# olivesgatech/R3D

Measured on AMD Instinct MI355X. Metric: training clips/sec (RGB+Depth fusion, DARai) at 1/2/4/8 GPUs; effective-rank match, higher is better.
Workload: dtype f32 (depth products: bf16x3 split on the bf16 matrix cores, fp32 accumulate)

## Files before the change

### include/r3d_hip.h

```cpp
#ifndef R3D_HIP_H
#define R3D_HIP_H

#include <stdint.h>

#ifdef __cplusplus
extern "C" {
#endif

#define R3D_ABI_VERSION 2

#define R3D_OK 0
#define R3D_EINVAL (-1)
#define R3D_EALIGN (-2)
#define R3D_ENORCCL (-3)
#define R3D_ERCCL_BASE (-100)

int r3d_abi_version(void);
int r3d_build_info(char* buf, int cap);

int r3d_allreduce_flat(float* buf, int64_t count, void* comm, void* stream);

#define R3D_GEMM_NT 0
#define R3D_GEMM_NN 1
#define R3D_GEMM_TN 2

typedef struct r3d_gemm_desc {
    const float* A; const float* B; float* C;
    int32_t layout, M, N, K;
    int32_t lda, ldb, ldc;
    const float* a_add; int32_t a_add_mod, a_add_ld, a_row_xor;
    const float* b_add; int32_t b_add_mod, b_add_ld;
    const float* bias;
    float* pre_out; int32_t ldpre;
    int32_t act;
    const uint8_t* drop_mask; int32_t lddrop; float drop_scale;
    const float* aux; int32_t ldaux, mul;
    const float* res1; int32_t ldr1;
    const float* res2; int32_t ldr2;
    float alpha; int32_t accumulate;
    float* bias_grad;
    int32_t c_row_xor;
    int32_t splitk, k_per_split; float* partial;
    int32_t tile;
    int32_t vec;
    float* adam_m; float* adam_v; const float* adam_lr; const int64_t* adam_step;
    float adam_beta1, adam_beta2, adam_eps, adam_wd, adam_gscale;
    int32_t prec;
} r3d_gemm_desc;

int r3d_gemm_f32(const r3d_gemm_desc* d, void* stream);
int r3d_splitk_reduce(const r3d_gemm_desc* d, void* stream);
int64_t r3d_gemm_partial_floats(int32_t M, int32_t N, int32_t splitk);
int r3d_gemm_bf3_nt_pair(const r3d_gemm_desc* first, const r3d_gemm_desc* second, void* stream);
int r3d_gemm_plan(r3d_gemm_desc* d);
int r3d_gemm_grouped_prepare(r3d_gemm_desc* descs, int n, int tile, int32_t* prefix);
int r3d_gemm_grouped_launch(const r3d_gemm_desc* dev_descs, const int32_t* dev_prefix, const int32_t* host_prefix, int n,
                            int total_tiles, int layout, int tile, void* stream);

int r3d_layernorm_fwd(const float* x, int ldx, int nsplit, const float* bias, float* pre_out, const float* gamma,
                      const float* beta, float* y, int ldy, float* mean, float* rstd, float* pair_out, int rows, int H,
                      int relu, void* stream);
int64_t r3d_layernorm_bwd_ws_floats(int rows, int H);
int r3d_layernorm_bwd(const float* dy, int lddy, int pair_in, const float* dy2, int lddy2, const float* x, int ldx,
                      const float* mean,
                      const float* rstd, const float* gamma, const float* beta, int relu, const float* add1, int ldadd1,
                      const float* add2, int ldadd2, float* dx, int lddx, float* dx2, int lddx2,
                      const uint8_t* drop_mask, int lddrop, float drop_scale, float* dgamma, float* dbeta, float* ws,
                      int rows, int H, int defer_finalize, void* stream);
int r3d_layernorm_bwd_finalize(const float* ws, int rows, int H, float* dgamma, float* dbeta, void* stream);
typedef struct r3d_ln_fwd_job {
    const float* x; int32_t ldx, nsplit; const float* bias; float* pre_out;
    const float* gamma; const float* beta; float* y; int32_t ldy; float* mean; float* rstd;
    float* pair_out; int32_t rows, H, relu;
} r3d_ln_fwd_job;
typedef struct r3d_ln_bwd_job {
    const float* dy; int32_t lddy, pair_in; const float* dy2; int32_t lddy2;
    const float* x; int32_t ldx; const float* mean; const float* rstd; const float* gamma; const float* beta; int32_t relu;
    const float* add1; int32_t ldadd1; const float* add2; int32_t ldadd2;
    float* dx; int32_t lddx;
    float* dx2; int32_t lddx2; const uint8_t* drop_mask; int32_t lddrop; float drop_scale;
    float* dgamma; float* dbeta; float* ws;
    int32_t rows, H, rows_per_block, nblocks;
} r3d_ln_bwd_job;
int r3d_layernorm_fwd_multi(const r3d_ln_fwd_job* jobs, int njobs, void* stream);
int r3d_layernorm_bwd_multi(r3d_ln_bwd_job* jobs, int njobs, void* stream);
typedef struct r3d_mha_bwd_job {
    const float* q; int32_t ldq; const float* k; int32_t ldk; const float* v; int32_t ldv;
    const float* probs; const uint8_t* drop_mask; float drop_scale;
    const float* d_o; int32_t lddo; float* dq; int32_t lddq; float* dk; int32_t lddk; float* dv; int32_t lddv;
    int32_t B, heads, Lq, Lk, dh;
} r3d_mha_bwd_job;
int r3d_layernorm_bwd_multi_mha(r3d_ln_bwd_job* jobs, int njobs, const r3d_mha_bwd_job* mha, void* stream);
typedef struct r3d_ln_finalize_job { const float* ws; float* dgamma; float* dbeta; int32_t rows, H; } r3d_ln_finalize_job;
int r3d_layernorm_bwd_finalize_batched(const r3d_ln_finalize_job* dev_jobs, int njobs, int max_H, void* stream);
int64_t r3d_colsum_ws_floats(int rows, int cols);
int r3d_colsum(const float* x, int ld, int rows, int cols, float* out, float* ws, int accumulate, void* stream);
int r3d_rowmod_sum(const float* x, int ld, int rows, int cols, int mod, float* out, int ldo, int accumulate,
                   void* stream);

typedef struct r3d_rowsum_job { const float* src1; const float* src2; float* dst; int32_t ld1, ld2, ldd, rows, cols, mod; } r3d_rowsum_job;
int r3d_rowmod_sum_batched(const r3d_rowsum_job* dev_jobs, int njobs, int max_cols, int max_mod, void* stream);
int r3d_tick(int64_t* a, int64_t* b, void* stream);
int r3d_add_rowbcast(const float* x, int ldx, const float* add, int ldadd, int mod, float* out, int ldo, int rows, int cols,
                     void* stream);

typedef struct r3d_gemm_ln_job {
    const float* A; int32_t lda;
    const float* W; int32_t ldw;
    const float* bias;
    const uint8_t* drop_mask; int32_t lddrop; float drop_scale;
    const float* res1; int32_t ldr1;
    const float* res2; int32_t ldr2;
    float* pre_out; int32_t ldpre;
    const float* gamma; const float* beta;
    float* y; int32_t ldy; float* mean; float* rstd;
    float* pair_out;
    int32_t M, K;
} r3d_gemm_ln_job;
int r3d_gemm_ln_supported(int M, int K, int H);
int r3d_gemm_ln_fwd(const r3d_gemm_ln_job* jobs, int njobs, int H, void* stream);
typedef struct r3d_mha_job {
    const float* q; int32_t ldq; const float* k; int32_t ldk; const float* v; int32_t ldv;
    const uint8_t* key_padding_mask; const int64_t* key_label; int32_t pad_idx;
    float* probs; const uint8_t* drop_mask; float drop_scale; float* o; int32_t ldo;
    int32_t B, heads, Lq, Lk, dh;
} r3d_mha_job;
int r3d_gemm_ln_mha_supported(int heads, int Lq, int Lk, int dh);
int r3d_gemm_ln_mha_fwd(const r3d_gemm_ln_job* jobs, int njobs, int H, const r3d_mha_job* mha, void* stream);

typedef struct r3d_fuser_chain_fwd_args {
    const float* x0; const float* h1;
    const float* wv; const float* wproj; const float* bproj; const float* g2; const float* be2;
    const float* w1; const float* b1; const float* w2; const float* b2; const float* gf; const float* bef;
    const float* pos; const float* wkv; const float* bkv; const float* wseg; const float* bseg;
    float* vsw; float* x1; float* h2; float* m2; float* r2; float* u; float* f1; float* x3; float* y; float* mf; float* rf;
    float* fused; float* seg; float* cakv;
    const float* qpos; const float* w_in; const float* b_in; const float* w_out; const float* b_out; const float* g1;
    const float* be1; const float* wq; const float* bq;
    const uint8_t* drop_sa; const uint8_t* drop_d1; float drop_scale;
    float* sa_qkv; float* p_sa; float* sa_o; float* t1_pre; float* t1; float* m1; float* r1; float* caq;
    int32_t N, S, K, H, add_xres, B, Q, heads;
    uint64_t* timeline;
    const uint16_t* pl_wv; const uint16_t* pl_wproj; const uint16_t* pl_w1; const uint16_t* pl_w2; const uint16_t* pl_wkv;
    const uint16_t* pl_wseg;
} r3d_fuser_chain_fwd_args;
typedef struct r3d_plane_job {
    const float* src; uint16_t* dst; int32_t ld, N, K, transposed, first_block, pad_;
} r3d_plane_job;
int64_t r3d_weight_plane_elems(int N, int K);
int r3d_weight_planes(const r3d_plane_job* jobs_device, int njobs, int total_blocks, void* stream);
int r3d_fuser_chain_supported(int N, int H, int K, int B, int Q, int heads);
int r3d_fuser_chain_fwd(const r3d_fuser_chain_fwd_args* a, void* stream);
typedef struct r3d_fuser_chain_bwd_args {
    const float* d_cakv; const float* d_seg; const float* d_extra; const float* wkv; const float* wseg;
    const float* x3; const float* mf; const float* rf; const float* gf;
    const float* w2; const float* u; const float* w1; const float* x1; const float* m2; const float* r2; const float* g2;
    const float* wproj; const float* wv; const float* x0; const float* m1; const float* r1; const float* g1n;
    const uint8_t* drop_x0; const float* m_rgb; const float* m_dep; const float* rgb; const float* dep_pre;
    const float* mean_d; const float* rstd_d; const float* lnd_g; const float* lnd_b;
    float* d_fused; float* d_x3; float* d_u; float* d_h2; float* d_x1; float* d_v; float* d_h1; float* d_rgb_pre;
    float* d_dep_pre; float* part_nf; float* part_n2; float* part_n1; float* part_dep;
    const float* d_caq; const float* d_t1_res; const float* wq; const float* t1_pre; const float* m1d; const float* r1d;
    const float* g1d; const uint8_t* drop_d1; const float* w_out; const float* sa_qkv; const float* p_sa;
    const uint8_t* drop_sa; const float* w_in;
    float* caqin; float* t1pre_out; float* sap; float* sao; float* saqkv; float* sain; float* part_d1;
    float drop_scale;
    int32_t N, S, K, H, add_xres, B, Q, heads;
    uint64_t* timeline;
    const uint16_t* pl_wkv_t; const uint16_t* pl_wseg_t; const uint16_t* pl_w2_t; const uint16_t* pl_w1_t;
    const uint16_t* pl_wproj_t; const uint16_t* pl_wv_t;
} r3d_fuser_chain_bwd_args;
int r3d_fuser_chain_bwd(const r3d_fuser_chain_bwd_args* a, void* stream);

int r3d_token_exchange3_fwd(const float* xa, const float* xb, const float* xc, const float* mask, const uint8_t* drop_mask,
                            float drop_scale, float* x0, int N, int C, void* stream);
int r3d_token_exchange3_bwd(const float* dx0, const float* mask, const uint8_t* drop_mask, float drop_scale, float* da, float* db,
                            float* dc, int N, int C, void* stream);
int r3d_attn3_fwd(const float* qkv, float* probs, float* out, int N, int C, int heads, void* stream);
int r3d_attn3_bwd(const float* qkv, const float* d_out, float* d_qkv, int N, int C, int heads, void* stream);
int r3d_triple_mean_fwd(const float* y, float* out, int N, int C, void* stream);
int r3d_triple_mean_bwd(const float* d_out, float* dy, int N, int C, void* stream);

int r3d_colabssum(const float* x, int ld, int rows, int cols, double* out, void* stream);
int r3d_token_select(const float* score_f, const double* score_sum, double count, int nvec, int C, int k,
                     int64_t* idx_out, float* mask_out, int* used_serial, void* stream);
int r3d_token_exchange_fwd(const float* rgb, const float* dep, const float* mask_rgb, const float* mask_dep, float* x0,
                           const uint8_t* drop_mask, float drop_scale, int N, int H, void* stream);
int r3d_token_exchange_bwd(const float* dx0, const float* rgb, const float* mask_rgb, const float* mask_dep,
                           const uint8_t* drop_mask, float drop_scale, float* d_rgb_pre, float* d_dep, int N, int H,
                           void* stream);

int r3d_mha_core_fwd(const float* q, int ldq, const float* k, int ldk, const float* v, int ldv,
                     const uint8_t* key_padding_mask, const int64_t* key_label, int pad_idx, float* probs,
                     const uint8_t* drop_mask, float drop_scale, float* o, int ldo, int B, int heads, int Lq, int Lk,
                     int dh, void* stream);
int r3d_mha_core_bwd(const float* q, int ldq, const float* k, int ldk, const float* v, int ldv, const float* probs,
                     const uint8_t* drop_mask, float drop_scale, const float* d_o, int lddo, float* dq, int lddq, float* dk,
                     int lddk, float* dv, int lddv, int B, int heads, int Lq, int Lk, int dh, void* stream);

#define R3D_DEC_FWD_NPTRS 57
int r3d_decoder_fused_supported(int S, int Q, int H, int heads);
int r3d_decoder_layer_fwd(const void* const* ptrs, int nptrs, int B, int S, int Q, int H, int heads, int pad_idx,
                          float drop_scale, int n_head_out, void* stream);

int r3d_embed_fuse_fwd(const float* rgb_src, int ns_r, const float* bias_r, const float* dep_src, int ns_d,
                       const float* bias_d, const float* lnd_gamma, const float* lnd_beta, const float* mask_rgb,
                       const float* mask_dep, const uint8_t* drop_mask, float drop_scale, const float* ln1_gamma,
                       const float* ln1_beta, float* rgb_out, float* dep_pre_out, float* mean_d, float* rstd_d,
                       float* dep_out, float* x0, float* h1, float* m1, float* r1, int N, int H, void* stream);
int r3d_embed_fuse_fwd_planes(const float* rgb_src, int ns_r, const float* bias_r, const float* dep_src, int ns_d,
                              const float* bias_d, const float* lnd_gamma, const float* lnd_beta, const float* mask_rgb,
                              const float* mask_dep, const uint8_t* drop_mask, float drop_scale, const float* ln1_gamma,
                              const float* ln1_beta, float* rgb_out, float* dep_pre_out, float* mean_d, float* rstd_d,
                              float* dep_out, float* x0, float* h1, float* m1, float* r1, int N, int H,
                              const r3d_plane_job* jobs_device, int njobs, int total_blocks, void* stream);
int r3d_embed_fuse_bwd(const float* d_h1, const float* x0, const float* m1, const float* r1, const float* ln1_gamma,
                       const float* add1, const float* add2, const uint8_t* drop_mask, float drop_scale,
                       const float* mask_rgb, const float* mask_dep, const float* rgb, const float* dep_pre,
                       const float* mean_d, const float* rstd_d, const float* lnd_gamma, const float* lnd_beta,
                       float* d_rgb_pre, float* d_dep_pre, float* ws_n1, float* ws_dep, int N, int H, void* stream);

int r3d_bn_stats(const float* x_rgb, const float* x_dep, float* run_mean_rgb, float* run_var_rgb, int64_t* nbt_rgb,
                 float* run_mean_dep, float* run_var_dep, int64_t* nbt_dep, const float* gamma_rgb, const float* gamma_dep,
                 float* mean, float* rstd, float* absgamma, int N, int C, int training, float momentum, void* stream);
int r3d_bn_blend_fwd(const float* rgb, const float* dep, const float* mean, const float* rstd, const float* gamma_rgb,
                     const float* beta_rgb, const float* gamma_dep, const float* beta_dep, const float* alpha,
                     const float* mask_rgb, const float* mask_dep, const uint8_t* drop_mask, float drop_scale,
                     const float* ln1_gamma, const float* ln1_beta, float* x0, float* h1, float* m1, float* r1, int N, int C,
                     void* stream);
int r3d_bn_blend_bwd(const float* d_h1, const float* x0, const float* m1, const float* r1, const float* ln1_gamma,
                     const float* add1, const uint8_t* drop_mask, float drop_scale, const float* rgb, const float* dep,
                     const float* mean, const float* rstd, const float* gamma_rgb, const float* beta_rgb,
                     const float* gamma_dep, const float* beta_dep, const float* alpha, const float* mask_rgb,
                     const float* mask_dep, float* t_drb, float* t_drbx, float* t_ddb, float* t_ddbx, float* t_dal,
                     float* ws_n1, int N, int C, void* stream);
int r3d_bn_bwd_apply(const float* rgb, const float* dep, const float* mean, const float* rstd, const float* gamma_rgb,
                     const float* gamma_dep, const float* t_drb, const float* t_ddb, const float* dgamma_rgb,
                     const float* dbeta_rgb, const float* dgamma_dep, const float* dbeta_dep, float* d_rgb_pre, float* d_dep,
                     int N, int C, int training, void* stream);
int r3d_bn_sync_pack(const float* mean, const float* rstd, int N, int C, float* out, void* stream);
int r3d_bn_sync_finalize(const float* all, int world, int n_local, int C, float* mean, float* rstd, float* run_mean_rgb,
                         float* run_var_rgb, int64_t* nbt_rgb, float* run_mean_dep, float* run_var_dep, int64_t* nbt_dep,
                         float* nfrac, float momentum, void* stream);

int r3d_decoder_tail_fwd(const float* x, const float* g3, const float* b3, const float* gF, const float* bF,
                         const float* w_head, const float* b_head, int n_head, float* t3, float* m3, float* r3, float* tgtF,
                         float* mF, float* rF, float* out, int ld_out, int rows, int H, void* stream);
int r3d_decoder_tail_bwd(const float* d_out, int ld_dout, const float* w_head, int n_head, const float* t3, const float* mF,
                         const float* rF, const float* gF, const float* x, const float* m3, const float* r3, const float* g3,
                         const uint8_t* drop_mask, float drop_scale, float* dx, float* dx2, float* dgF, float* dbF,
                         float* dg3, float* db3, float* wsF, float* ws3, int rows, int H, void* stream);

int r3d_losses_fwd_bwd(const float* seg_logits, int ld_seg, const float* act_logits, int ld_act, const float* dur,
                       int ld_dur, const int64_t* past_label, const int64_t* target, const float* target_dur, int B, int S,
                       int Q, int K, int pad_idx, int exclude_idx, int val_mode, const float* dur_den, float grad_scale,
                       float* d_seg, int ld_dseg, float* d_act, int ld_dact, float* d_dur, int ld_ddur, float* loss_out,
                       int64_t* counts, float* ws, int64_t* tick_a, int64_t* tick_b, void* stream);
int64_t r3d_losses_ws_floats(int B, int S, int Q);

typedef struct r3d_tail_losses_args {
    const float* x; const float* g3; const float* b3; const float* gF; const float* bF;
    const float* w_head; const float* b_head; int n_head;
    float* t3; float* m3; float* r3; float* tgtF; float* mF; float* rF; float* out; int ld_out; int H;
    const float* seg; int ld_seg; const int64_t* past_label; const int64_t* target; const float* target_dur;
    int B, S, Q, K, pad_idx, exclude_idx; const float* dur_den; float grad_scale;
    float* d_seg; int ld_dseg; float* d_out; int ld_dout; float* loss_out; int64_t* counts; int64_t* tick_a; int64_t* tick_b;
    const uint8_t* drop; float drop_scale; float* dx; float* dx2; float* wsF; float* ws3;
    int defer_finalize;
} r3d_tail_losses_args;
int r3d_decoder_tail_losses_supported(int H, int n_head, int Q, int rows);
int r3d_decoder_tail_losses(const r3d_tail_losses_args* a, float* ws, void* stream);

typedef struct r3d_decoder_chain_args {
    const float* caq; const float* cakv; const int64_t* key_label; float* p_ca; const uint8_t* drop_ca; float* ca_o;
    const float* wo; const float* bo; const uint8_t* drop_d2; const float* t1; float* t2_pre; const float* g2; const float* be2;
    float* t2; float* m2; float* r2; const float* w1; const float* b1; const uint8_t* drop_ff; float* ff1;
    const float* w2; const float* b2; const uint8_t* drop_d3; float* t3_pre;
    const float* d_t3pre; const float* d_ff2; float* d_ff1; float* d_t2pre; float* d_cap; float* d_cao; float* d_caq;
    float* d_cakv; float* part_d2;
    float drop_scale;
    int32_t pad_idx, B, S, H, Q, heads, phases;
    uint64_t* timeline;
    const uint16_t* pl_wo; const uint16_t* pl_w1; const uint16_t* pl_w2; const uint16_t* pl_w2_t; const uint16_t* pl_w1_t;
    const uint16_t* pl_wo_t;
} r3d_decoder_chain_args;
int r3d_decoder_chain_supported(int H, int Q, int heads, int S);
int r3d_decoder_chain(const r3d_decoder_chain_args* d, const r3d_tail_losses_args* tail, float* ws, void* stream);

int r3d_adamw_flat(float* p, const float* g, float* m, float* v, int64_t n, const float* lr, const int64_t* step,
                   float beta1, float beta2, float eps, float weight_decay, float grad_scale, void* stream);
int r3d_adamw_flat_dropout(float* p, const float* g, float* m, float* v, int64_t n, const float* lr, const int64_t* step,
                           float beta1, float beta2, float eps, float weight_decay, float grad_scale, uint8_t* mask,
                           int64_t n_mask, float p_drop, uint64_t seed, const int64_t* offset, void* stream);
typedef struct r3d_loss_finalize_job {
    const float* part; int32_t B, S, Q, has_seg;
    const float* dur_den;
    float* loss_out; int64_t* counts;
    double* acc_loss; int64_t* acc_counts;
} r3d_loss_finalize_job;
int r3d_losses_finalize(const r3d_loss_finalize_job* job, void* stream);
int r3d_adamw_flat_fin(float* p, const float* g, float* m, float* v, int64_t n, const float* lr, const int64_t* step,
                       float beta1, float beta2, float eps, float weight_decay, float grad_scale,
                       const r3d_loss_finalize_job* fin, void* stream);
int r3d_adamw_flat_dropout_fin(float* p, const float* g, float* m, float* v, int64_t n, const float* lr, const int64_t* step,
                               float beta1, float beta2, float eps, float weight_decay, float grad_scale, uint8_t* mask,
                               int64_t n_mask, float p_drop, uint64_t seed, const int64_t* offset,
                               const r3d_loss_finalize_job* fin, void* stream);
int r3d_adamw_2d(float* p, const float* g, float* m, float* v, int rows, int cols, int ld, const float* lr,
                 const int64_t* step, float beta1, float beta2, float eps, float weight_decay, float grad_scale, void* stream);
int r3d_dropout_mask(uint8_t* mask, int64_t n, float p, uint64_t seed, const int64_t* offset, void* stream);

int64_t r3d_erank_lds_bytes(int R, int C);
int r3d_erank_jacobi(const float* x, int ld, int64_t batch_stride, int batch, int R, int C, int gram, float* sigma,
                     float* af_t, float* stats, int max_sweeps, void* stream);
int r3d_erank_blocked_sizes(int R, int C, int max_sweeps, int64_t* out);
int r3d_erank_blocked(const float* x, int ld, int R, int C, float* sigma, float* af_t, int* ctrl, float* stats,
                      int max_sweeps, void* stream);
int r3d_erank_blocked_t(const float* x, int ld, int x_transposed, int R, int C, float* sigma, float* af_t, int* ctrl,
                        float* stats, int max_sweeps, void* stream);
int r3d_erank_bwd_coef(const float* sigma, const float* stats, const float* gout, float* coef, int C, int max_rank,
                       void* stream);
int r3d_scale_rows(float* x, int ld, int rows, int cols, const float* coef, void* stream);
int r3d_erank_bwd_coef2(const float* sigma, const float* stats, const float* gout, float* cg, float* inv, int C, int max_rank,
                        void* stream);
int r3d_erank_bwd_fix(float* w, const float* p, const float* cg, int rows, int cols, void* stream);
int64_t r3d_erank_lds_bytes_v(int R, int C);
int r3d_erank_jacobi_warm(const float* x, int ld, int64_t batch_stride, int batch, int R, int C, int gram, float* sigma,
                          float* af_t, float* stats, int max_sweeps, const float* vt_in, float* vt_out, void* stream);
int r3d_erank_vt_polish(const float* vt_raw, const float* gv, float* vt, int64_t n, void* stream);

int r3d_posenc_fwd(const float* x, int ldx, const float* table, int ldt, int S, const uint8_t* drop, float drop_scale,
                   float* y, int ldy, int rows, int H, void* stream);
int r3d_posenc_bwd(const float* dy, int lddy, const uint8_t* drop, float drop_scale, const float* gate, int ldg, float* dx,
                   int lddx, int rows, int H, void* stream);
int r3d_avgpool_rows_fwd(const float* x, int ldx, float* y, int ldy, int B, int S, int Q, int H, void* stream);
int r3d_avgpool_rows_bwd(const float* dy, int lddy, float* dx, int lddx, int B, int S, int Q, int H, void* stream);
int r3d_embed_gather_fwd(const float* weight, int n_embed, const int64_t* idx, const float* table, int ldt, int S, float* out,
                         int ldo, int rows, int H, void* stream);
int r3d_embed_gather_bwd(const float* d_out, int ldd, const int64_t* idx, float* d_weight, int n_embed, int rows, int H,
                         void* stream);

typedef struct r3d_clip_collate_job {
    const float* rgb_pool; int64_t F_rgb, D;
    const float* depth_pool; int64_t F_dep, P;
    int64_t n_items;
    const int64_t* off_f; const int64_t* ids_f;
    const int64_t* off_d; const int64_t* ids_d;
    const int64_t* off_l; const int64_t* lab;
    const int64_t* off_q; const float* q_dur; const int64_t* q_tgt;
    const int64_t* items; int64_t B;
    int64_t S_f, S_d, S_l, S_q, pad_idx;
    float* features; float* depth; int64_t* past_label; float* trans_future_dur; int64_t* trans_future_target;
} r3d_clip_collate_job;
int r3d_clip_collate(const r3d_clip_collate_job* job, void* stream);

#ifdef __cplusplus
}
#endif
#endif
```

### r3d_amd/_lib.py

```python
import ctypes as C
import os

HERE = os.path.dirname(os.path.abspath(__file__))
LIB_PATH = os.path.join(HERE, "_build", "libr3d_hip.so")
ABI_VERSION = 2

c_float_p = C.c_void_p


class GemmDesc(C.Structure):
    _fields_ = [
        ("A", C.c_void_p), ("B", C.c_void_p), ("C", C.c_void_p),
        ("layout", C.c_int32), ("M", C.c_int32), ("N", C.c_int32), ("K", C.c_int32),
        ("lda", C.c_int32), ("ldb", C.c_int32), ("ldc", C.c_int32),
        ("a_add", C.c_void_p), ("a_add_mod", C.c_int32), ("a_add_ld", C.c_int32), ("a_row_xor", C.c_int32),
        ("b_add", C.c_void_p), ("b_add_mod", C.c_int32), ("b_add_ld", C.c_int32),
        ("bias", C.c_void_p),
        ("pre_out", C.c_void_p), ("ldpre", C.c_int32),
        ("act", C.c_int32),
        ("drop_mask", C.c_void_p), ("lddrop", C.c_int32), ("drop_scale", C.c_float),
        ("aux", C.c_void_p), ("ldaux", C.c_int32), ("mul", C.c_int32),
        ("res1", C.c_void_p), ("ldr1", C.c_int32),
        ("res2", C.c_void_p), ("ldr2", C.c_int32),
        ("alpha", C.c_float), ("accumulate", C.c_int32),
        ("bias_grad", C.c_void_p),
        ("c_row_xor", C.c_int32),
        ("splitk", C.c_int32), ("k_per_split", C.c_int32), ("partial", C.c_void_p),
        ("tile", C.c_int32),
        ("vec", C.c_int32),
        ("adam_m", C.c_void_p), ("adam_v", C.c_void_p), ("adam_lr", C.c_void_p), ("adam_step", C.c_void_p),
        ("adam_beta1", C.c_float), ("adam_beta2", C.c_float), ("adam_eps", C.c_float), ("adam_wd", C.c_float),
        ("adam_gscale", C.c_float),
        ("prec", C.c_int32),
    ]


class LnFwdJob(C.Structure):
    _fields_ = [("x", C.c_void_p), ("ldx", C.c_int32), ("nsplit", C.c_int32), ("bias", C.c_void_p), ("pre_out", C.c_void_p),
                ("gamma", C.c_void_p), ("beta", C.c_void_p), ("y", C.c_void_p), ("ldy", C.c_int32), ("mean", C.c_void_p),
                ("rstd", C.c_void_p), ("pair_out", C.c_void_p), ("rows", C.c_int32), ("H", C.c_int32), ("relu", C.c_int32)]


class LnBwdJob(C.Structure):
    _fields_ = [("dy", C.c_void_p), ("lddy", C.c_int32), ("pair_in", C.c_int32), ("dy2", C.c_void_p), ("lddy2", C.c_int32),
                ("x", C.c_void_p), ("ldx", C.c_int32), ("mean", C.c_void_p), ("rstd", C.c_void_p), ("gamma", C.c_void_p),
                ("beta", C.c_void_p), ("relu", C.c_int32), ("add1", C.c_void_p), ("ldadd1", C.c_int32), ("add2", C.c_void_p),
                ("ldadd2", C.c_int32), ("dx", C.c_void_p), ("lddx", C.c_int32), ("dx2", C.c_void_p), ("lddx2", C.c_int32),
                ("drop_mask", C.c_void_p), ("lddrop", C.c_int32), ("drop_scale", C.c_float), ("dgamma", C.c_void_p),
                ("dbeta", C.c_void_p), ("ws", C.c_void_p), ("rows", C.c_int32), ("H", C.c_int32),
                ("rows_per_block", C.c_int32), ("nblocks", C.c_int32)]


class GemmLnJob(C.Structure):
    _fields_ = [("A", C.c_void_p), ("lda", C.c_int32), ("W", C.c_void_p), ("ldw", C.c_int32), ("bias", C.c_void_p),
                ("drop_mask", C.c_void_p), ("lddrop", C.c_int32), ("drop_scale", C.c_float),
                ("res1", C.c_void_p), ("ldr1", C.c_int32), ("res2", C.c_void_p), ("ldr2", C.c_int32),
                ("pre_out", C.c_void_p), ("ldpre", C.c_int32), ("gamma", C.c_void_p), ("beta", C.c_void_p),
                ("y", C.c_void_p), ("ldy", C.c_int32), ("mean", C.c_void_p), ("rstd", C.c_void_p),
                ("pair_out", C.c_void_p), ("M", C.c_int32), ("K", C.c_int32)]


class FuserChainFwdArgs(C.Structure):
    _PTRS = ("x0 h1 wv wproj bproj g2 be2 w1 b1 w2 b2 gf bef pos wkv bkv wseg bseg vsw x1 h2 m2 r2 u f1 x3 y mf rf fused seg "
             "cakv qpos w_in b_in w_out b_out g1 be1 wq bq drop_sa drop_d1").split()
    _PTRS2 = "sa_qkv p_sa sa_o t1_pre t1 m1 r1 caq".split()
    _PLANES = "pl_wv pl_wproj pl_w1 pl_w2 pl_wkv pl_wseg".split()
    _fields_ = ([(n, C.c_void_p) for n in _PTRS] + [("drop_scale", C.c_float)] + [(n, C.c_void_p) for n in _PTRS2] +
                [(n, C.c_int32) for n in "N S K H add_xres B Q heads".split()] + [("timeline", C.c_void_p)] +
                [(n, C.c_void_p) for n in _PLANES])


class PlaneJob(C.Structure):
    _fields_ = [("src", C.c_void_p), ("dst", C.c_void_p), ("ld", C.c_int32), ("N", C.c_int32), ("K", C.c_int32),
                ("transposed", C.c_int32), ("first_block", C.c_int32), ("pad_", C.c_int32)]


class FuserChainBwdArgs(C.Structure):
    _PTRS = ("d_cakv d_seg d_extra wkv wseg x3 mf rf gf w2 u w1 x1 m2 r2 g2 wproj wv x0 m1 r1 g1n drop_x0 m_rgb m_dep rgb "
             "dep_pre mean_d rstd_d lnd_g lnd_b d_fused d_x3 d_u d_h2 d_x1 d_v d_h1 d_rgb_pre d_dep_pre part_nf part_n2 "
             "part_n1 part_dep d_caq d_t1_res wq t1_pre m1d r1d g1d drop_d1 w_out sa_qkv p_sa drop_sa w_in caqin t1pre_out "
             "sap sao saqkv sain part_d1").split()
    _PLANES = "pl_wkv_t pl_wseg_t pl_w2_t pl_w1_t pl_wproj_t pl_wv_t".split()
    _fields_ = ([(n, C.c_void_p) for n in _PTRS] + [("drop_scale", C.c_float)] +
                [(n, C.c_int32) for n in "N S K H add_xres B Q heads".split()] + [("timeline", C.c_void_p)] +
                [(n, C.c_void_p) for n in _PLANES])


class DecoderChainArgs(C.Structure):
    _PTRS = ("caq cakv key_label p_ca drop_ca ca_o wo bo drop_d2 t1 t2_pre g2 be2 t2 m2 r2 w1 b1 drop_ff ff1 w2 b2 drop_d3 "
             "t3_pre d_t3pre d_ff2 d_ff1 d_t2pre d_cap d_cao d_caq d_cakv part_d2").split()
    _fields_ = ([(n, C.c_void_p) for n in _PTRS] + [("drop_scale", C.c_float)] +
                [(n, C.c_int32) for n in "pad_idx B S H Q heads phases".split()] + [("timeline", C.c_void_p)] +
                [(n, C.c_void_p) for n in "pl_wo pl_w1 pl_w2 pl_w2_t pl_w1_t pl_wo_t".split()])


class MhaJob(C.Structure):
    _fields_ = [("q", C.c_void_p), ("ldq", C.c_int32), ("k", C.c_void_p), ("ldk", C.c_int32), ("v", C.c_void_p),
                ("ldv", C.c_int32), ("key_padding_mask", C.c_void_p), ("key_label", C.c_void_p), ("pad_idx", C.c_int32),
                ("probs", C.c_void_p), ("drop_mask", C.c_void_p), ("drop_scale", C.c_float), ("o", C.c_void_p),
                ("ldo", C.c_int32), ("B", C.c_int32), ("heads", C.c_int32), ("Lq", C.c_int32), ("Lk", C.c_int32),
                ("dh", C.c_int32)]


class MhaBwdJob(C.Structure):
    _fields_ = [("q", C.c_void_p), ("ldq", C.c_int32), ("k", C.c_void_p), ("ldk", C.c_int32), ("v", C.c_void_p),
                ("ldv", C.c_int32), ("probs", C.c_void_p), ("drop_mask", C.c_void_p), ("drop_scale", C.c_float),
                ("d_o", C.c_void_p), ("lddo", C.c_int32), ("dq", C.c_void_p), ("lddq", C.c_int32), ("dk", C.c_void_p),
                ("lddk", C.c_int32), ("dv", C.c_void_p), ("lddv", C.c_int32), ("B", C.c_int32), ("heads", C.c_int32),
                ("Lq", C.c_int32), ("Lk", C.c_int32), ("dh", C.c_int32)]


class RowsumJob(C.Structure):
    _fields_ = [("src1", C.c_void_p), ("src2", C.c_void_p), ("dst", C.c_void_p), ("ld1", C.c_int32), ("ld2", C.c_int32),
                ("ldd", C.c_int32), ("rows", C.c_int32), ("cols", C.c_int32), ("mod", C.c_int32)]


class TailLossesArgs(C.Structure):
    _fields_ = ([(n, C.c_void_p) for n in ("x", "g3", "b3", "gF", "bF", "w_head", "b_head")] + [("n_head", C.c_int32)] +
                [(n, C.c_void_p) for n in ("t3", "m3", "r3", "tgtF", "mF", "rF", "out")] +
                [("ld_out", C.c_int32), ("H", C.c_int32), ("seg", C.c_void_p), ("ld_seg", C.c_int32),
                 ("past_label", C.c_void_p), ("target", C.c_void_p), ("target_dur", C.c_void_p)] +
                [(n, C.c_int32) for n in ("B", "S", "Q", "K", "pad_idx", "exclude_idx")] +
                [("dur_den", C.c_void_p), ("grad_scale", C.c_float), ("d_seg", C.c_void_p), ("ld_dseg", C.c_int32),
                 ("d_out", C.c_void_p), ("ld_dout", C.c_int32), ("loss_out", C.c_void_p), ("counts", C.c_void_p),
                 ("tick_a", C.c_void_p), ("tick_b", C.c_void_p), ("drop", C.c_void_p), ("drop_scale", C.c_float)] +
                [(n, C.c_void_p) for n in ("dx", "dx2", "wsF", "ws3")] + [("defer_finalize", C.c_int32)])


class LossFinalizeJob(C.Structure):
    _fields_ = [("part", C.c_void_p), ("B", C.c_int32), ("S", C.c_int32), ("Q", C.c_int32), ("has_seg", C.c_int32),
                ("dur_den", C.c_void_p), ("loss_out", C.c_void_p), ("counts", C.c_void_p), ("acc_loss", C.c_void_p),
                ("acc_counts", C.c_void_p)]


class LnFinalizeJob(C.Structure):
    _fields_ = [("ws", C.c_void_p), ("dgamma", C.c_void_p), ("dbeta", C.c_void_p), ("rows", C.c_int32), ("H", C.c_int32)]


class ClipCollateJob(C.Structure):
    _fields_ = ([("rgb_pool", C.c_void_p), ("F_rgb", C.c_int64), ("D", C.c_int64),
                 ("depth_pool", C.c_void_p), ("F_dep", C.c_int64), ("P", C.c_int64), ("n_items", C.c_int64)] +
                [(n, C.c_void_p) for n in "off_f ids_f off_d ids_d off_l lab off_q q_dur q_tgt items".split()] +
                [(n, C.c_int64) for n in "B S_f S_d S_l S_q pad_idx".split()] +
                [(n, C.c_void_p) for n in "features depth past_label trans_future_dur trans_future_target".split()])


GEMM_NT, GEMM_NN, GEMM_TN = 0, 1, 2

_I, _L, _F, _P, _D = C.c_int, C.c_int64, C.c_float, C.c_void_p, C.c_double

_SIGNATURES = {
    "r3d_abi_version": ([], C.c_int),
    "r3d_build_info": ([C.c_char_p, _I], C.c_int),
    "r3d_allreduce_flat": ([_P, _L, _P, _P], C.c_int),
    "r3d_gemm_f32": ([C.POINTER(GemmDesc), _P], C.c_int),
    "r3d_splitk_reduce": ([C.POINTER(GemmDesc), _P], C.c_int),
    "r3d_gemm_partial_floats": ([C.c_int32, C.c_int32, C.c_int32], C.c_int64),
    "r3d_gemm_plan": ([C.POINTER(GemmDesc)], C.c_int),
    "r3d_gemm_grouped_prepare": ([C.POINTER(GemmDesc), _I, _I, C.POINTER(C.c_int32)], C.c_int),
    "r3d_gemm_grouped_launch": ([_P, _P, C.POINTER(C.c_int32), _I, _I, _I, _I, _P], C.c_int),
    "r3d_gemm_ln_supported": ([_I, _I, _I], C.c_int),
    "r3d_gemm_ln_fwd": ([_P, _I, _I, _P], C.c_int),
    "r3d_fuser_chain_supported": ([_I, _I, _I, _I, _I, _I], C.c_int),
    "r3d_fuser_chain_fwd": ([_P, _P], C.c_int),
    "r3d_fuser_chain_bwd": ([_P, _P], C.c_int),
    "r3d_weight_plane_elems": ([_I, _I], C.c_int64),
    "r3d_weight_planes": ([_P, _I, _I, _P], C.c_int),
    "r3d_token_exchange3_fwd": ([_P, _P, _P, _P, _P, _F, _P, _I, _I, _P], C.c_int),
    "r3d_token_exchange3_bwd": ([_P, _P, _P, _F, _P, _P, _P, _I, _I, _P], C.c_int),
    "r3d_attn3_fwd": ([_P, _P, _P, _I, _I, _I, _P], C.c_int),
    "r3d_attn3_bwd": ([_P, _P, _P, _I, _I, _I, _P], C.c_int),
    "r3d_triple_mean_fwd": ([_P, _P, _I, _I, _P], C.c_int),
    "r3d_triple_mean_bwd": ([_P, _P, _I, _I, _P], C.c_int),
    "r3d_decoder_chain_supported": ([_I, _I, _I, _I], C.c_int),
    "r3d_decoder_chain": ([_P, _P, _P, _P], C.c_int),
    "r3d_gemm_ln_mha_supported": ([_I, _I, _I, _I], C.c_int),
    "r3d_gemm_ln_mha_fwd": ([_P, _I, _I, _P, _P], C.c_int),
    "r3d_layernorm_fwd_multi": ([_P, _I, _P], C.c_int),
    "r3d_layernorm_bwd_multi": ([_P, _I, _P], C.c_int),
    "r3d_layernorm_bwd_multi_mha": ([_P, _I, _P, _P], C.c_int),
    "r3d_layernorm_bwd_finalize_batched": ([_P, _I, _I, _P], C.c_int),
    "r3d_layernorm_fwd": ([_P, _I, _I, _P, _P, _P, _P, _P, _I, _P, _P, _P, _I, _I, _I, _P], C.c_int),
    "r3d_layernorm_bwd_ws_floats": ([_I, _I], C.c_int64),
    "r3d_add_rowbcast": ([_P, _I, _P, _I, _I, _P, _I, _I, _I, _P], C.c_int),
    "r3d_layernorm_bwd": ([_P, _I, _I, _P, _I, _P, _I, _P, _P, _P, _P, _I, _P, _I, _P, _I, _P, _I, _P, _I, _P, _I, _F,
                           _P, _P, _P, _I, _I, _I, _P], C.c_int),
    "r3d_layernorm_bwd_finalize": ([_P, _I, _I, _P, _P, _P], C.c_int),
    "r3d_colsum_ws_floats": ([_I, _I], C.c_int64),
    "r3d_colsum": ([_P, _I, _I, _I, _P, _P, _I, _P], C.c_int),
    "r3d_rowmod_sum": ([_P, _I, _I, _I, _I, _P, _I, _I, _P], C.c_int),
    "r3d_rowmod_sum_batched": ([_P, _I, _I, _I, _P], C.c_int),
    "r3d_tick": ([_P, _P, _P], C.c_int),
    "r3d_colabssum": ([_P, _I, _I, _I, _P, _P], C.c_int),
    "r3d_token_select": ([_P, _P, _D, _I, _I, _I, _P, _P, _P, _P], C.c_int),
    "r3d_token_exchange_fwd": ([_P, _P, _P, _P, _P, _P, _F, _I, _I, _P], C.c_int),
    "r3d_token_exchange_bwd": ([_P, _P, _P, _P, _P, _F, _P, _P, _I, _I, _P], C.c_int),
    "r3d_mha_core_fwd": ([_P, _I, _P, _I, _P, _I, _P, _P, _I, _P, _P, _F, _P, _I, _I, _I, _I, _I, _I, _P], C.c_int),
    "r3d_mha_core_bwd": ([_P, _I, _P, _I, _P, _I, _P, _P, _F, _P, _I, _P, _I, _P, _I, _P, _I, _I, _I, _I, _I, _I, _P],
                         C.c_int),
    "r3d_decoder_fused_supported": ([_I, _I, _I, _I], C.c_int),
    "r3d_decoder_layer_fwd": ([_P, _I, _I, _I, _I, _I, _I, _I, _F, _I, _P], C.c_int),
    "r3d_embed_fuse_fwd": ([_P, _I, _P, _P, _I, _P, _P, _P, _P, _P, _P, _F, _P, _P, _P, _P, _P, _P, _P, _P, _P, _P, _P, _I, _I,
                            _P], C.c_int),
    "r3d_gemm_bf3_nt_pair": ([_P, _P, _P], C.c_int),
    "r3d_embed_fuse_fwd_planes": ([_P, _I, _P, _P, _I, _P, _P, _P, _P, _P, _P, _F, _P, _P, _P, _P, _P, _P, _P, _P, _P, _P, _P, _I,
                                   _I, _P, _I, _I, _P], C.c_int),
    "r3d_embed_fuse_bwd": ([_P, _P, _P, _P, _P, _P, _P, _P, _F, _P, _P, _P, _P, _P, _P, _P, _P, _P, _P, _P, _P, _I, _I, _P],
                           C.c_int),
    "r3d_bn_stats": ([_P] * 13 + [_I, _I, _I, _F, _P], C.c_int),
    "r3d_bn_blend_fwd": ([_P] * 12 + [_F] + [_P] * 6 + [_I, _I, _P], C.c_int),
    "r3d_bn_blend_bwd": ([_P] * 7 + [_F] + [_P] * 17 + [_I, _I, _P], C.c_int),
    "r3d_bn_bwd_apply": ([_P] * 14 + [_I, _I, _I, _P], C.c_int),
    "r3d_bn_sync_pack": ([_P, _P, _I, _I, _P, _P], C.c_int),
    "r3d_bn_sync_finalize": ([_P, _I, _I, _I] + [_P] * 9 + [_F, _P], C.c_int),
    "r3d_decoder_tail_fwd": ([_P, _P, _P, _P, _P, _P, _P, _I, _P, _P, _P, _P, _P, _P, _P, _I, _I, _I, _P], C.c_int),
    "r3d_decoder_tail_bwd": ([_P, _I, _P, _I, _P, _P, _P, _P, _P, _P, _P, _P, _P, _F, _P, _P, _P, _P, _P, _P, _P, _P, _I, _I,
                              _P], C.c_int),
    "r3d_decoder_tail_losses_supported": ([_I, _I, _I, _I], C.c_int),
    "r3d_decoder_tail_losses": ([_P, _P, _P], C.c_int),
    "r3d_losses_fwd_bwd": ([_P, _I, _P, _I, _P, _I, _P, _P, _P, _I, _I, _I, _I, _I, _I, _I, _P, _F, _P, _I, _P, _I,
                            _P, _I, _P, _P, _P, _P, _P, _P], C.c_int),
    "r3d_losses_ws_floats": ([_I, _I, _I], C.c_int64),
    "r3d_adamw_flat": ([_P, _P, _P, _P, _L, _P, _P, _F, _F, _F, _F, _F, _P], C.c_int),
    "r3d_adamw_flat_dropout": ([_P, _P, _P, _P, _L, _P, _P, _F, _F, _F, _F, _F, _P, _L, _F, C.c_uint64, _P, _P], C.c_int),
    "r3d_losses_finalize": ([_P, _P], C.c_int),
    "r3d_adamw_flat_fin": ([_P, _P, _P, _P, _L, _P, _P, _F, _F, _F, _F, _F, _P, _P], C.c_int),
    "r3d_adamw_flat_dropout_fin": ([_P, _P, _P, _P, _L, _P, _P, _F, _F, _F, _F, _F, _P, _L, _F, C.c_uint64, _P, _P, _P], C.c_int),
    "r3d_adamw_2d": ([_P, _P, _P, _P, _I, _I, _I, _P, _P, _F, _F, _F, _F, _F, _P], C.c_int),
    "r3d_dropout_mask": ([_P, _L, _F, C.c_uint64, _P, _P], C.c_int),
    "r3d_erank_lds_bytes": ([_I, _I], C.c_int64),
    "r3d_erank_jacobi": ([_P, _I, _L, _I, _I, _I, _I, _P, _P, _P, _I, _P], C.c_int),
    "r3d_erank_blocked_sizes": ([_I, _I, _I, _P], C.c_int),
    "r3d_erank_blocked": ([_P, _I, _I, _I, _P, _P, _P, _P, _I, _P], C.c_int),
    "r3d_erank_blocked_t": ([_P, _I, _I, _I, _I, _P, _P, _P, _P, _I, _P], C.c_int),
    "r3d_erank_bwd_coef": ([_P, _P, _P, _P, _I, _I, _P], C.c_int),
    "r3d_erank_bwd_coef2": ([_P, _P, _P, _P, _P, _I, _I, _P], C.c_int),
    "r3d_erank_bwd_fix": ([_P, _P, _P, _I, _I, _P], C.c_int),
    "r3d_scale_rows": ([_P, _I, _I, _I, _P, _P], C.c_int),
    "r3d_posenc_fwd": ([_P, _I, _P, _I, _I, _P, _F, _P, _I, _I, _I, _P], C.c_int),
    "r3d_posenc_bwd": ([_P, _I, _P, _F, _P, _I, _P, _I, _I, _I, _P], C.c_int),
    "r3d_avgpool_rows_fwd": ([_P, _I, _P, _I, _I, _I, _I, _I, _P], C.c_int),
    "r3d_avgpool_rows_bwd": ([_P, _I, _P, _I, _I, _I, _I, _I, _P], C.c_int),
    "r3d_embed_gather_fwd": ([_P, _I, _P, _P, _I, _I, _P, _I, _I, _I, _P], C.c_int),
    "r3d_embed_gather_bwd": ([_P, _I, _P, _P, _I, _I, _I, _P], C.c_int),
    "r3d_erank_lds_bytes_v": ([_I, _I], C.c_int64),
    "r3d_erank_jacobi_warm": ([_P, _I, _L, _I, _I, _I, _I, _P, _P, _P, _I, _P, _P, _P], C.c_int),
    "r3d_erank_vt_polish": ([_P, _P, _P, _L, _P], C.c_int),
    "r3d_clip_collate": ([C.POINTER(ClipCollateJob), _P], C.c_int),
}

EXPORTS = tuple(_SIGNATURES)

_lib = None


class R3DHipError(RuntimeError):
    pass


def load():
    global _lib
    if _lib is not None:
        return _lib
    if not os.path.exists(LIB_PATH):
        raise R3DHipError(
            f"{LIB_PATH} is missing: the HIP kernels are the only compute path of r3d_amd (no CPU/PyTorch fallback). "
            f"Build it with `python -m r3d_amd.build` (needs hipcc; cross-compiles for gfx950 without a GPU).")
    lib = C.CDLL(LIB_PATH)
    for name, (argt, rest) in _SIGNATURES.items():
        try:
            fn = getattr(lib, name)
        except AttributeError as e:
            raise R3DHipError(f"{LIB_PATH} does not export {name}: stale build, run `python -m r3d_amd.build --force`") from e
        fn.argtypes = argt
        fn.restype = rest
    v = lib.r3d_abi_version()
    if v != ABI_VERSION:
        raise R3DHipError(f"libr3d_hip.so ABI {v} != expected {ABI_VERSION}: rebuild with `python -m r3d_amd.build --force`")
    _lib = lib
    return lib


_ERR = {-1: "R3D_EINVAL (rejected argument)", -2: "R3D_EALIGN (misaligned pointer / leading dimension)",
        -3: "R3D_ENORCCL (no RCCL mapped into the process)"}


def check(rc, what):
    if rc <= -100:
        raise R3DHipError(f"{what} failed: ncclResult_t {-100 - rc} from RCCL")
    if rc != 0:
        raise R3DHipError(f"{what} failed: {_ERR.get(rc, f'hipError_t {rc}' if rc > 0 else rc)}")


def build_info():
    buf = C.create_string_buffer(128)
    check(load().r3d_build_info(buf, 128), "r3d_build_info")
    return buf.value.decode()
```

### r3d_amd/csrc/decoder_chain.hip

```cpp
#include "chain_bf3.h"
#include "mha_small.h"
#include "losses_dev.h"

namespace r3d {

constexpr int kDcBufA = 0;
constexpr int kDcBufB = kDcBufA + kFcRows * kFcP1;
constexpr int kDcBufF = kDcBufB + kFcRows * kFcP1;
constexpr int kDcWl = kDcBufF + kFcRows * kFcP4;
constexpr int kDcWlWave = 128 * kFbWP;
constexpr int kDcRed = kDcWl + 8 * kDcWlWave;
constexpr int kDcLdsFloats = kDcRed + 2 * 2 * 8 * kFcRows;
constexpr int kDcLdsBytes = kDcLdsFloats * 4;
static_assert(16 * kFcWP <= kDcWlWave && mha_small_lds_floats(16, 8) <= kDcWlWave && mha_small_bwd_lds_floats(16, 8) <= kDcWlWave,
              "wave region");
static_assert(kDcLdsBytes + (2 * 8 * (kTLHeads + 8) + 8 * 4 * 128 + 64) * 4 <= 160 * 1024, "LDS (dynamic + the tail's static arrays)");

typedef r3d_decoder_chain_args DcArgs;

__device__ __forceinline__ void dc_stage_rows(float* buf, const float* src, int row0, int tid) {
    const int r = tid >> 5, c4 = tid & 31;
    const f32x4 z = {0.f, 0.f, 0.f, 0.f};
    const f32x4 v = *reinterpret_cast<const f32x4*>(src + (size_t)(row0 + (r & 7)) * kFcH + 4 * c4);
    *reinterpret_cast<f32x4*>(buf + r * kFcP1 + 4 * c4) = r < 8 ? v : z;
// ... 123 lines not shown
    }
}

__device__ __forceinline__ void dc_bwd(const DcArgs& D, const int b, float* lds) {
    const int tid = threadIdx.x, lane = tid & 63, wave = tid >> 6;
    const int li = lane & 15, q = lane >> 4;
    float* bufA = lds + kDcBufA;
    float* bufF = lds + kDcBufF;
    float* wl = lds + kDcWl + wave * kDcWlWave;
    float* redA = lds + kDcRed;
    constexpr int H = kFcH;
    const int row0 = b * 8;
    const int c = wave * 16 + li, n0 = wave * 16;
    const bool live = q < 2;
    const f32x4 zero = {0.f, 0.f, 0.f, 0.f};
    R3D_CHAIN_MARK(D.timeline, b == 0, 10);
    FcW s0, s1;
    fb_wload(s0, D.w2 + (4 * wave + 0) * 16, 4 * H, 128, lane);
    fb_wload(s1, D.w2 + (4 * wave + 1) * 16, 4 * H, 128, lane);
    dc_stage_rows(bufA, D.d_ff2, row0, tid);
    const FcMaskSrc md2(D.drop_d2, D.g2, H), mff(D.drop_ff, D.g2, 4 * H);
    float ffv[4][4], res[4], t2pv[4], m2v[4], r2v[4];
    uint8_t kb2[4], kbf[4][4];
#pragma unroll
    for (int i = 0; i < 4; ++i) {
        const size_t r = (size_t)(row0 + ((4 * q + i) & 7));
#pragma unroll
        for (int t = 0; t < 4; ++t) {
            ffv[t][i] = D.ff1[r * (4 * H) + (4 * wave + t) * 16 + li];
            kbf[t][i] = mff.raw(r, (4 * wave + t) * 16 + li);
        }
        res[i] = D.d_t3pre[r * H + c];
        t2pv[i] = D.t2_pre[r * H + c];
        m2v[i] = D.m2[r]; r2v[i] = D.r2[r];
        kb2[i] = md2.raw(r, c);
    }
    const float g2 = D.g2[c];
    __builtin_amdgcn_sched_barrier(0);
    fb_wstore(s0, wl, lane);
    fb_wload(s0, D.w2 + (4 * wave + 2) * 16, 4 * H, 128, lane);
    __syncthreads();
    FcOp a;
    f32x4 acc0, acc1;
    R3D_CHAIN_MARK(D.timeline, b == 0, 11);
    fc_opload(a, bufA + li * kFcP1 + 4 * q);
#pragma unroll
    for (int t = 0; t < 4; ++t) {
        acc0 = zero; acc1 = zero;
        fb_chunk(a, wl, li, q, acc0, acc1);
        __builtin_amdgcn_sched_barrier(0);
        if (t == 0) { fb_wstore(s1, wl, lane); fb_wload(s1, D.w2 + (4 * wave + 3) * 16, 4 * H, 128, lane); }
        if (t == 1) { fb_wstore(s0, wl, lane); fb_wload(s0, D.w1 + n0, H, 128, lane); }
        if (t == 2) { fb_wstore(s1, wl, lane); fb_wload(s1, D.w1 + (size_t)128 * H + n0, H, 128, lane); }
        if (t == 3) { fb_wstore(s0, wl, lane); fb_wload(s0, D.w1 + (size_t)256 * H + n0, H, 128, lane); }
        __builtin_amdgcn_sched_barrier(0);
        const int cu = (4 * wave + t) * 16 + li;
#pragma unroll
        for (int i = 0; i < 4; ++i) {
            const float gv = ffv[t][i] > 0.f ? (acc0[i] + acc1[i]) * mff.keep(kbf[t][i], D.drop_scale) : 0.f;
            if (live) D.d_ff1[(size_t)(row0 + 4 * q + i) * (4 * H) + cu] = gv;
            bufF[(4 * q + i) * kFcP4 + cu] = live ? gv : 0.f;
        }
    }
    __syncthreads();
    R3D_CHAIN_MARK(D.timeline, b == 0, 12);
    acc0 = zero; acc1 = zero;
    const float* ar = bufF + li * kFcP4 + 4 * q;
    fc_opload(a, ar);
    fb_chunk(a, wl, li, q, acc0, acc1);
    __builtin_amdgcn_sched_barrier(0);
    fb_wstore(s1, wl, lane);
    fb_wload(s1, D.w1 + (size_t)384 * H + n0, H, 128, lane);
    __builtin_amdgcn_sched_barrier(0);
    fc_opload(a, ar + 128);
    fb_chunk(a, wl, li, q, acc0, acc1);
    __builtin_amdgcn_sched_barrier(0);
    fb_wstore(s0, wl, lane);
    fb_wload(s0, D.wo + n0, H, 128, lane);
    __builtin_amdgcn_sched_barrier(0);
    fc_opload(a, ar + 256);
    fb_chunk(a, wl, li, q, acc0, acc1);
    __builtin_amdgcn_sched_barrier(0);
    fb_wstore(s1, wl, lane);
    __builtin_amdgcn_sched_barrier(0);
    fc_opload(a, ar + 384);
    fb_chunk(a, wl, li, q, acc0, acc1);
    __builtin_amdgcn_sched_barrier(0);
    fb_wstore(s0, wl, lane);
    __builtin_amdgcn_sched_barrier(0);
    {
        float d[4], xh[4], g[4], gx[4], s1v[4], s2v[4];
#pragma unroll
        for (int i = 0; i < 4; ++i) {
            d[i] = live ? (acc0[i] + acc1[i]) + res[i] : 0.f;
            xh[i] = (t2pv[i] - m2v[i]) * r2v[i];
            g[i] = d[i] * g2;
            gx[i] = g[i] * xh[i];
        }
        if (live) {
            float* pp = D.part_d2 + (size_t)(2 * b + q) * (2 * H);
            pp[c] = (d[0] * xh[0] + d[1] * xh[1]) + (d[2] * xh[2] + d[3] * xh[3]);
            pp[H + c] = (d[0] + d[1]) + (d[2] + d[3]);
        }
        fb_rowsum2<4>(g, gx, redA, wave, li, q, s1v, s2v);
#pragma unroll
        for (int i = 0; i < 4; ++i) {
            const float o = r2v[i] * (g[i] - s1v[i] - xh[i] * s2v[i]);
            const size_t e = (size_t)(row0 + 4 * q + i) * H + c;
            const float ok = o * md2.keep(kb2[i], D.drop_scale);
            if (live) { D.d_t2pre[e] = o; D.d_cap[e] = ok; }
            bufA[(4 * q + i) * kFcP1 + c] = live ? ok : 0.f;
        }
    }
    __syncthreads();
    R3D_CHAIN_MARK(D.timeline, b == 0, 13);
    fc_opload(a, bufA + li * kFcP1 + 4 * q);
    acc0 = zero; acc1 = zero;
    fb_chunk(a, wl, li, q, acc0, acc1);
    if (live) {
#pragma unroll
        for (int i = 0; i < 4; ++i) D.d_cao[(size_t)(row0 + 4 * q + i) * H + c] = acc0[i] + acc1[i];
    }
    R3D_CHAIN_MARK(D.timeline, b == 0, 14);
    __syncthreads();
    {
        MhaArgs m{};
        m.q = D.caq; m.ldq = H; m.k = D.cakv; m.ldk = 2 * H; m.v = D.cakv + H; m.ldv = 2 * H;
        m.probs = D.p_ca; m.drop = D.drop_ca; m.drop_scale = D.drop_scale; m.d_o = D.d_cao; m.lddo = H;
        m.dq = D.d_caq; m.lddq = H; m.dk = D.d_cakv; m.lddk = 2 * H; m.dv = D.d_cakv + H; m.lddv = 2 * H;
        m.B = D.B; m.heads = 8; m.Lq = 8; m.Lk = D.S; m.dh = 16; m.scale = 0.25f;
        mha_bwd_small_unit<16, 8, false>(m, b * 8 + wave, wl);
    }
    R3D_CHAIN_MARK(D.timeline, b == 0, 15);
}

constexpr int kD3P1 = kFcH + 8, kD3P4 = 4 * kFcH + 8;
constexpr int kD3ImgA = 0;
constexpr int kD3ImgB = kD3ImgA + 3 * 16 * kD3P1;
constexpr int kD3ImgF = kD3ImgB + 3 * 16 * kD3P1;
constexpr int kD3ScrBytes = (kD3ImgF + 3 * 16 * kD3P4) * 2;
constexpr int kD3ScrWave = 1856;
constexpr int kD3RedBytes = kD3ScrBytes + 8 * kD3ScrWave * 4;
constexpr int kD3LdsBytes = kD3RedBytes + 2 * 2 * 8 * kFcRows * 4;
static_assert(mha_small_lds_floats(16, 8) <= kD3ScrWave && mha_small_bwd_lds_floats(16, 8) <= kD3ScrWave, "attention scratch");
static_assert(kD3LdsBytes + (2 * 8 * (kTLHeads + 8) + 8 * 4 * 128 + 64) * 4 <= 160 * 1024, "LDS (dynamic + the tail's static arrays)");

__device__ __forceinline__ void dc3_stage_rows(unsigned short* img, const float* src, int row0, int tid) {
    const int r = tid >> 5, c4 = tid & 31;
    const f32x4 z = {0.f, 0.f, 0.f, 0.f};
    const f32x4 v = *reinterpret_cast<const f32x4*>(src + (size_t)(row0 + (r & 7)) * kFcH + 4 * c4);
    bf3_store4(img, kD3P1, r, 4 * c4, r < 8 ? v : z);
}

__device__ __forceinline__ void dc3_fwd(const DcArgs& D, const int b, float* lds) {
    const int tid = threadIdx.x, lane = tid & 63, wave = tid >> 6;
    const int li = lane & 15, q = lane >> 4;
    unsigned short* img = reinterpret_cast<unsigned short*>(lds);
    unsigned short* imgA = img + kD3ImgA;
    unsigned short* imgB = img + kD3ImgB;
    unsigned short* imgF = img + kD3ImgF;
    float* scr = reinterpret_cast<float*>(reinterpret_cast<unsigned char*>(lds) + kD3ScrBytes) + wave * kD3ScrWave;
    float (*red)[8][kFcRows] = reinterpret_cast<float (*)[8][kFcRows]>(reinterpret_cast<unsigned char*>(lds) + kD3RedBytes);
    constexpr int H = kFcH;
    const int row0 = b * 8;
    const int c = wave * 16 + li;
    const bool live = q < 2;
    const f32x4 zero = {0.f, 0.f, 0.f, 0.f};
    R3D_CHAIN_MARK(D.timeline, b == 0, 0);
    Bf3B b0, b1, b2;
    bf3_bload<4>(b0, D.pl_wo, 4, wave, 0, lane);
    bf3_bload<4>(b1, D.pl_w1, 4, 4 * wave + 0, 0, lane);
    bf3_bload<4>(b2, D.pl_w1, 4, 4 * wave + 1, 0, lane);
    const FcMaskSrc md2(D.drop_d2, D.g2, H), md3(D.drop_d3, D.g2, H), mff(D.drop_ff, D.g2, 4 * H);
    float t1v[4];
    uint8_t kb2[4], kb3[4], kbf[4][4];
#pragma unroll
    for (int i = 0; i < 4; ++i) {
        const size_t r = (size_t)(row0 + ((4 * q + i) & 7));
        t1v[i] = D.t1[r * H + c];
        kb2[i] = md2.raw(r, c);
        kb3[i] = md3.raw(r, c);
#pragma unroll
        for (int t = 0; t < 4; ++t) kbf[t][i] = mff.raw(r, (4 * wave + t) * 16 + li);
    }
    const float b_o = D.bo[c], g2 = D.g2[c], be2 = D.be2[c], b_2 = D.b2[c];
    float b_1[4];
#pragma unroll
    for (int t = 0; t < 4; ++t) b_1[t] = D.b1[(4 * wave + t) * 16 + li];
    R3D_CHAIN_MARK(D.timeline, b == 0, 1);
    {
        MhaArgs m{};
        m.q = D.caq; m.ldq = H; m.k = D.cakv; m.ldk = 2 * H; m.v = D.cakv + H; m.ldv = 2 * H;
        m.key_label = D.key_label; m.pad_idx = D.pad_idx; m.probs = D.p_ca; m.drop = D.drop_ca; m.drop_scale = D.drop_scale;
        m.o = D.ca_o; m.ldo = H; m.B = D.B; m.heads = 8; m.Lq = 8; m.Lk = D.S; m.dh = 16; m.scale = 0.25f;
        mha_fwd_small_unit<16, 8, false>(m, b * 8 + wave, scr);
    }
    R3D_CHAIN_MARK(D.timeline, b == 0, 2);
    __syncthreads();
    dc3_stage_rows(imgA, D.ca_o, row0, tid);
    __syncthreads();
    R3D_CHAIN_MARK(D.timeline, b == 0, 3);
    f32x4 acc0 = zero, acc1 = zero;
    bf3_chunk<4>(imgA, kD3P1, li, q, 0, b0, acc0, acc1);
    __builtin_amdgcn_sched_barrier(0);
    bf3_bload<4>(b0, D.pl_w1, 4, 4 * wave + 2, 0, lane);
    __builtin_amdgcn_sched_barrier(0);
    float t2p[4], mean[4], rstd[4], t2v[4];
#pragma unroll
    for (int i = 0; i < 4; ++i) {
        t2p[i] = ((acc0[i] + acc1[i]) + b_o) * md2.keep(kb2[i], D.drop_scale) + t1v[i];
        if (live) D.t2_pre[(size_t)(row0 + 4 * q + i) * H + c] = t2p[i];
    }
    fc_layernorm(t2p, red, wave, li, q, mean, rstd);
#pragma unroll
    for (int i = 0; i < 4; ++i) {
        t2v[i] = (t2p[i] - mean[i]) * rstd[i] * g2 + be2;
        const int r = 4 * q + i;
        if (live) {
            D.t2[(size_t)(row0 + r) * H + c] = t2v[i];
            if (wave == 0 && li == 0) { D.m2[row0 + r] = mean[i]; D.r2[row0 + r] = rstd[i]; }
        }
        bf3_store1(imgB, kD3P1, r, c, live ? t2v[i] : 0.f);
    }
    __syncthreads();
    R3D_CHAIN_MARK(D.timeline, b == 0, 4);
#pragma unroll
    for (int t = 0; t < 4; ++t) {
        acc0 = zero; acc1 = zero;
        if (t == 0) bf3_chunk<4>(imgB, kD3P1, li, q, 0, b1, acc0, acc1);
        if (t == 1) bf3_chunk<4>(imgB, kD3P1, li, q, 0, b2, acc0, acc1);
        if (t == 2) bf3_chunk<4>(imgB, kD3P1, li, q, 0, b0, acc0, acc1);
        if (t == 3) bf3_chunk<4>(imgB, kD3P1, li, q, 0, b1, acc0, acc1);
        __builtin_amdgcn_sched_barrier(0);
        if (t == 0) bf3_bload<4>(b1, D.pl_w1, 4, 4 * wave + 3, 0, lane);
        if (t == 1) bf3_bload<4>(b2, D.pl_w2, 16, wave, 0, lane);
        if (t == 2) bf3_bload<4>(b0, D.pl_w2, 16, wave, 4, lane);
        if (t == 3) bf3_bload<4>(b1, D.pl_w2, 16, wave, 8, lane);
        __builtin_amdgcn_sched_barrier(0);
        const int cu = (4 * wave + t) * 16 + li;
#pragma unroll
        for (int i = 0; i < 4; ++i) {
            const float f = fmaxf((acc0[i] + acc1[i]) + b_1[t], 0.f) * mff.keep(kbf[t][i], D.drop_scale);
            if (live) D.ff1[(size_t)(row0 + 4 * q + i) * (4 * H) + cu] = f;
            bf3_store1(imgF, kD3P4, 4 * q + i, cu, live ? f : 0.f);
        }
    }
    __syncthreads();
    R3D_CHAIN_MARK(D.timeline, b == 0, 5);
    acc0 = zero; acc1 = zero;
    bf3_chunk<4>(imgF, kD3P4, li, q, 0, b2, acc0, acc1);
    __builtin_amdgcn_sched_barrier(0);
    bf3_bload<4>(b2, D.pl_w2, 16, wave, 12, lane);
    __builtin_amdgcn_sched_barrier(0);
    bf3_chunk<4>(imgF, kD3P4, li, q, 4, b0, acc0, acc1);
    bf3_chunk<4>(imgF, kD3P4, li, q, 8, b1, acc0, acc1);
    bf3_chunk<4>(imgF, kD3P4, li, q, 12, b2, acc0, acc1);
    if (live) {
#pragma unroll
        for (int i = 0; i < 4; ++i)
            D.t3_pre[(size_t)(row0 + 4 * q + i) * H + c] =
                ((acc0[i] + acc1[i]) + b_2) * md3.keep(kb3[i], D.drop_scale) + t2v[i];
    }
}

__device__ __forceinline__ void dc3_bwd(const DcArgs& D, const int b, float* lds) {
    const int tid = threadIdx.x, lane = tid & 63, wave = tid >> 6;
    const int li = lane & 15, q = lane >> 4;
    unsigned short* img = reinterpret_cast<unsigned short*>(lds);
    unsigned short* imgA = img + kD3ImgA;
    unsigned short* imgF = img + kD3ImgF;
    float* scr = reinterpret_cast<float*>(reinterpret_cast<unsigned char*>(lds) + kD3ScrBytes) + wave * kD3ScrWave;
    float* redA = reinterpret_cast<float*>(reinterpret_cast<unsigned char*>(lds) + kD3RedBytes);
    constexpr int H = kFcH;
    const int row0 = b * 8;
    const int c = wave * 16 + li;
    const bool live = q < 2;
    const f32x4 zero = {0.f, 0.f, 0.f, 0.f};
    R3D_CHAIN_MARK(D.timeline, b == 0, 10);
    Bf3B b0, b1, b2;
    bf3_bload<4>(b0, D.pl_w2_t, 4, 4 * wave + 0, 0, lane);
    bf3_bload<4>(b1, D.pl_w2_t, 4, 4 * wave + 1, 0, lane);
    bf3_bload<4>(b2, D.pl_w2_t, 4, 4 * wave + 2, 0, lane);
    dc3_stage_rows(imgA, D.d_ff2, row0, tid);
    const FcMaskSrc md2(D.drop_d2, D.g2, H), mff(D.drop_ff, D.g2, 4 * H);
    float ffv[4][4], res[4], t2pv[4], m2v[4], r2v[4];
    uint8_t kb2[4], kbf[4][4];
#pragma unroll
    for (int i = 0; i < 4; ++i) {
        const size_t r = (size_t)(row0 + ((4 * q + i) & 7));
#pragma unroll
        for (int t = 0; t < 4; ++t) {
            ffv[t][i] = D.ff1[r * (4 * H) + (4 * wave + t) * 16 + li];
            kbf[t][i] = mff.raw(r, (4 * wave + t) * 16 + li);
        }
        res[i] = D.d_t3pre[r * H + c];
        t2pv[i] = D.t2_pre[r * H + c];
        m2v[i] = D.m2[r]; r2v[i] = D.r2[r];
        kb2[i] = md2.raw(r, c);
    }
    const float g2 = D.g2[c];
    __syncthreads();
    R3D_CHAIN_MARK(D.timeline, b == 0, 11);
    f32x4 acc0, acc1;
#pragma unroll
    for (int t = 0; t < 4; ++t) {
        acc0 = zero; acc1 = zero;
        if (t == 0) bf3_chunk<4>(imgA, kD3P1, li, q, 0, b0, acc0, acc1);
        if (t == 1) bf3_chunk<4>(imgA, kD3P1, li, q, 0, b1, acc0, acc1);
        if (t == 2) bf3_chunk<4>(imgA, kD3P1, li, q, 0, b2, acc0, acc1);
        if (t == 3) bf3_chunk<4>(imgA, kD3P1, li, q, 0, b0, acc0, acc1);
        __builtin_amdgcn_sched_barrier(0);
        if (t == 0) bf3_bload<4>(b0, D.pl_w2_t, 4, 4 * wave + 3, 0, lane);
        if (t == 1) bf3_bload<4>(b1, D.pl_w1_t, 16, wave, 0, lane);
        if (t == 2) bf3_bload<4>(b2, D.pl_w1_t, 16, wave, 4, lane);
        if (t == 3) bf3_bload<4>(b0, D.pl_w1_t, 16, wave, 8, lane);
        __builtin_amdgcn_sched_barrier(0);
        const int cu = (4 * wave + t) * 16 + li;
#pragma unroll
        for (int i = 0; i < 4; ++i) {
            const float gv = ffv[t][i] > 0.f ? (acc0[i] + acc1[i]) * mff.keep(kbf[t][i], D.drop_scale) : 0.f;
            if (live) D.d_ff1[(size_t)(row0 + 4 * q + i) * (4 * H) + cu] = gv;
            bf3_store1(imgF, kD3P4, 4 * q + i, cu, live ? gv : 0.f);
        }
    }
    __syncthreads();
    R3D_CHAIN_MARK(D.timeline, b == 0, 12);
    acc0 = zero; acc1 = zero;
    bf3_chunk<4>(imgF, kD3P4, li, q, 0, b1, acc0, acc1);
    __builtin_amdgcn_sched_barrier(0);
    bf3_bload<4>(b1, D.pl_w1_t, 16, wave, 12, lane);
    __builtin_amdgcn_sched_barrier(0);
    bf3_chunk<4>(imgF, kD3P4, li, q, 4, b2, acc0, acc1);
    __builtin_amdgcn_sched_barrier(0);
    bf3_bload<4>(b2, D.pl_wo_t, 4, wave, 0, lane);
    __builtin_amdgcn_sched_barrier(0);
    bf3_chunk<4>(imgF, kD3P4, li, q, 8, b0, acc0, acc1);
    bf3_chunk<4>(imgF, kD3P4, li, q, 12, b1, acc0, acc1);
    {
        float d[4], xh[4], g[4], gx[4], s1v[4], s2v[4];
#pragma unroll
        for (int i = 0; i < 4; ++i) {
            d[i] = live ? (acc0[i] + acc1[i]) + res[i] : 0.f;
            xh[i] = (t2pv[i] - m2v[i]) * r2v[i];
            g[i] = d[i] * g2;
            gx[i] = g[i] * xh[i];
        }
        if (live) {
            float* pp = D.part_d2 + (size_t)(2 * b + q) * (2 * H);
            pp[c] = (d[0] * xh[0] + d[1] * xh[1]) + (d[2] * xh[2] + d[3] * xh[3]);
            pp[H + c] = (d[0] + d[1]) + (d[2] + d[3]);
        }
        fb_rowsum2<4>(g, gx, redA, wave, li, q, s1v, s2v);
#pragma unroll
        for (int i = 0; i < 4; ++i) {
            const float o = r2v[i] * (g[i] - s1v[i] - xh[i] * s2v[i]);
            const size_t e = (size_t)(row0 + 4 * q + i) * H + c;
            const float ok = o * md2.keep(kb2[i], D.drop_scale);
            if (live) { D.d_t2pre[e] = o; D.d_cap[e] = ok; }
            bf3_store1(imgA, kD3P1, 4 * q + i, c, live ? ok : 0.f);
        }
    }
    __syncthreads();
    R3D_CHAIN_MARK(D.timeline, b == 0, 13);
    acc0 = zero; acc1 = zero;
    bf3_chunk<4>(imgA, kD3P1, li, q, 0, b2, acc0, acc1);
    if (live) {
#pragma unroll
        for (int i = 0; i < 4; ++i) D.d_cao[(size_t)(row0 + 4 * q + i) * H + c] = acc0[i] + acc1[i];
    }
    R3D_CHAIN_MARK(D.timeline, b == 0, 14);
    __syncthreads();
    {
        MhaArgs m{};
        m.q = D.caq; m.ldq = H; m.k = D.cakv; m.ldk = 2 * H; m.v = D.cakv + H; m.ldv = 2 * H;
        m.probs = D.p_ca; m.drop = D.drop_ca; m.drop_scale = D.drop_scale; m.d_o = D.d_cao; m.lddo = H;
        m.dq = D.d_caq; m.lddq = H; m.dk = D.d_cakv; m.lddk = 2 * H; m.dv = D.d_cakv + H; m.lddv = 2 * H;
        m.B = D.B; m.heads = 8; m.Lq = 8; m.Lk = D.S; m.dh = 16; m.scale = 0.25f;
        mha_bwd_small_unit<16, 8, false>(m, b * 8 + wave, scr);
    }
    R3D_CHAIN_MARK(D.timeline, b == 0, 15);
}

__global__ __launch_bounds__(512) void decoder_chain_bf3_kernel(const DcArgs D, const r3d_tail_losses_args t, const LossArgs a,
                                                                float* part, unsigned* arrivals) {
    extern __shared__ __attribute__((aligned(16))) float lds[];
    __shared__ float lg[8][kTLHeads + 8];
    __shared__ float dl[8][kTLHeads + 8];
    __shared__ float red[8][4][128];
    __shared__ int is_last;
    if (threadIdx.x >= 256) __builtin_amdgcn_s_setprio(0); else __builtin_amdgcn_s_setprio(2);
    const int lane = threadIdx.x & 63, wave = threadIdx.x >> 6;
    if ((int)blockIdx.x < D.B) {
        const int b = (int)blockIdx.x;
        if (D.phases & 1) dc3_fwd(D, b, lds);
        R3D_CHAIN_MARK(D.timeline, b == 0, 6);
        if (D.phases & 2) {
            __syncthreads();
            tail_clip_body(t, a, part, b, lg, dl, red);
        }
        R3D_CHAIN_MARK(D.timeline, b == 0, 7);
        if (D.phases & 4) {
            __syncthreads();
            dc3_bwd(D, b, lds);
        }
    } else if (D.phases & 2) {
        const int u = ((int)blockIdx.x - D.B) * 8 + wave;
        if (u < a.B * a.S) losses_unit(a, part, u, lane);
    }
    if (D.phases & 2) tail_losses_finish(t, a, part, arrivals, &is_last);
}

__global__ __launch_bounds__(512) void decoder_chain_kernel(const DcArgs D, const r3d_tail_losses_args t, const LossArgs a,
                                                            float* part, unsigned* arrivals) {
    extern __shared__ __attribute__((aligned(16))) float lds[];
    if (threadIdx.x >= 256) __builtin_amdgcn_s_setprio(0); else __builtin_amdgcn_s_setprio(2);
    __shared__ float lg[8][kTLHeads + 8];
    __shared__ float dl[8][kTLHeads + 8];
    __shared__ float red[8][4][128];
    __shared__ int is_last;
    const int lane = threadIdx.x & 63, wave = threadIdx.x >> 6;
    if ((int)blockIdx.x < D.B) {
        const int b = (int)blockIdx.x;
        if (D.phases & 1) dc_fwd(D, b, lds);
        R3D_CHAIN_MARK(D.timeline, b == 0, 6);
        if (D.phases & 2) {
            __syncthreads();
            tail_clip_body(t, a, part, b, lg, dl, red);
        }
        R3D_CHAIN_MARK(D.timeline, b == 0, 7);
        if (D.phases & 4) {
            __syncthreads();
            dc_bwd(D, b, lds);
        }
    } else if (D.phases & 2) {
        const int u = ((int)blockIdx.x - D.B) * 8 + wave;
        if (u < a.B * a.S) losses_unit(a, part, u, lane);
    }
    if (D.phases & 2) tail_losses_finish(t, a, part, arrivals, &is_last);
}

}

using namespace r3d;

R3D_EXPORT int r3d_decoder_tail_losses_supported(int H, int n_head, int Q, int rows);

R3D_EXPORT int r3d_decoder_chain_supported(int H, int Q, int heads, int S) {
    return (H == kFcH && Q == 8 && heads == 8 && S > 0 && S <= 64) ? 1 : 0;
}

R3D_EXPORT int r3d_decoder_chain(const r3d_decoder_chain_args* d, const r3d_tail_losses_args* tail, float* ws, void* stream) {
    R3D_REQUIRE(d && (d->phases & 7) && !(d->phases & ~7));
    R3D_REQUIRE(r3d_decoder_chain_supported(d->H, d->Q, d->heads, d->S) && d->B > 0);
    R3D_REQUIRE(d->caq && d->cakv && d->p_ca && d->wo && d->w1 && d->w2 && d->t2_pre && d->m2 && d->r2 && d->g2 && d->ff1);
    if (d->phases & 1)
        R3D_REQUIRE(d->ca_o && d->bo && d->t1 && d->be2 && d->t2 && d->b1 && d->b2 && d->t3_pre);
    if (d->phases & 4)
        R3D_REQUIRE(d->d_t3pre && d->d_ff2 && d->d_ff1 && d->d_t2pre && d->d_cap && d->d_cao && d->d_caq && d->d_cakv && d->part_d2);
    const void* al[] = {d->caq, d->cakv, d->wo, d->w1, d->w2, d->ca_o, d->d_ff2, d->d_cao, d->d_cakv};
    for (const void* p : al)
        if (p && !r3d_aligned16(p)) return R3D_EALIGN;
    r3d_tail_losses_args t{};
    LossArgs a{};
    int grid = d->B;
    unsigned* arrivals = nullptr;
    if (d->phases & 2) {
        R3D_REQUIRE(tail && ws);
        t = *tail;
        R3D_REQUIRE(t.x && t.g3 && t.b3 && t.gF && t.bF && t.w_head && t.b_head && t.t3 && t.m3 && t.r3 && t.tgtF && t.mF && t.rF);
        R3D_REQUIRE(t.out && t.seg && t.past_label && t.target && t.target_dur && t.d_seg && t.d_out && t.loss_out && t.counts);
        R3D_REQUIRE(t.dx && t.dx2 && t.wsF && t.ws3);
        R3D_REQUIRE(t.B == d->B && t.S == d->S && t.Q == d->Q && t.H == d->H && t.K > 0 && t.n_head == t.K + 1);
        R3D_REQUIRE(t.ld_out >= t.n_head && t.ld_dout >= t.n_head && t.ld_seg >= t.K && t.ld_dseg >= t.K);
        if (!r3d_decoder_tail_losses_supported(t.H, t.n_head, t.Q, t.B * t.Q)) return R3D_EINVAL;
        if (!r3d_aligned16(ws)) return R3D_EALIGN;
        if (d->phases & 1) R3D_REQUIRE(t.x == d->t3_pre);
        if (d->phases & 4) R3D_REQUIRE(t.dx == d->d_t3pre && t.dx2 == d->d_ff2);
        a = LossArgs{t.seg, t.ld_seg, t.out, t.ld_out, t.out + t.K, t.ld_out, t.past_label, t.target, t.target_dur, t.B, t.S, t.Q,
                     t.K, t.pad_idx, t.exclude_idx, 0, t.dur_den, t.grad_scale, t.d_seg, t.ld_dseg, t.d_out, t.ld_dout,
                     t.d_out + t.K, t.ld_dout, t.loss_out, t.counts, t.tick_a, t.tick_b};
        const int units = t.B * t.S + t.B * t.Q + t.B;
        grid = t.B + r3d_cdiv(t.B * t.S, 8);
        arrivals = reinterpret_cast<unsigned*>(ws + 4 * (size_t)units);
    }
    if (d->pl_wo) {
        R3D_REQUIRE(d->pl_w1 && d->pl_w2 && d->pl_w2_t && d->pl_w1_t && d->pl_wo_t);
        hipError_t e3 = hipFuncSetAttribute((const void*)decoder_chain_bf3_kernel, hipFuncAttributeMaxDynamicSharedMemorySize,
                                            kD3LdsBytes);
        if (e3 != hipSuccess) return (int)e3;
        hipLaunchKernelGGL(decoder_chain_bf3_kernel, dim3(grid), dim3(512), (size_t)kD3LdsBytes, (hipStream_t)stream, *d, t, a, ws,
                           arrivals);
        R3D_LAUNCH_CHECK();
        return R3D_OK;
    }
    hipError_t e = hipFuncSetAttribute((const void*)decoder_chain_kernel, hipFuncAttributeMaxDynamicSharedMemorySize, kDcLdsBytes);
    if (e != hipSuccess) return (int)e;
    hipLaunchKernelGGL(decoder_chain_kernel, dim3(grid), dim3(512), (size_t)kDcLdsBytes, (hipStream_t)stream, *d, t, a, ws, arrivals);
    R3D_LAUNCH_CHECK();
    return R3D_OK;
}
```

### r3d_amd/engine.py

```python
import math

import torch

from . import ops
from ._lib import GEMM_NT, GEMM_NN, GEMM_TN

LIVE_PREFIXES = ("input_embed.", "depth_projection.", "depth_layernorm.", "pos_embedding", "query_embed.",
                 "fuser.blocks.", "fuser.norm.", "transformer.decoder.", "fc_seg.", "fc.", "fc_len.")
EXCLUDE_CLASS_IDX = 47
DROP_P = 0.1


BN_LIVE_PREFIXES = ("fuser.alpha", "fuser.bn_rgb.", "fuser.bn_depth.")


def is_live(name):
    return name.startswith(LIVE_PREFIXES)


BWD_BF3_MAX_K = 32


def fuser_chain_shape_ok(B, S, H, K, Q, heads, bn=False):
    return bool(not bn and H // heads == 16 and ops.fuser_chain_supported(B * S, H, K, B, Q, heads))


def decoder_chain_shape_ok(B, S, H, Q, heads, L):
    return bool(L == 1 and H // heads == 16 and B * Q <= 1024 and ops.decoder_chain_supported(H, Q, heads, S))


def bwd_chain_bf3(chain_bf3, K):
    return bool(chain_bf3 and K <= BWD_BF3_MAX_K)


def tail_in_decoder_chain(B, H, K, Q):
    return ops.tail_losses_supported(H, K + 1, Q, B * Q)


class ParamArena:

    def __init__(self, named_params, device, extra_live=()):
        named = list(named_params)
        self.is_live = lambda n: is_live(n) or (bool(extra_live) and n.startswith(tuple(extra_live)))
        live = [(n, p) for n, p in named if self.is_live(n)]
        dead = [(n, p) for n, p in named if not self.is_live(n)]

        def key(item):
            n, p = item
            if n == "depth_projection.weight":
                return (3, 0)
            if n in ("fc.weight", "fc_len.weight"):
                return (0, 0 if n == "fc.weight" else 1)
            if n in ("fc.bias", "fc_len.bias"):
                return (2, 0 if n == "fc.bias" else 1)
            if n == "pos_embedding":
                return (2, 9)
            return (1, 0) if p.numel() % 4 == 0 else (2, 2)
        order = sorted(range(len(live)), key=lambda i: (key(live[i]), i))
        live = [live[i] for i in order]
        self.offsets, off = {}, 0
        for n, p in live:
            if n in ("depth_projection.weight", "pos_embedding"):
                off = (off + 3) // 4 * 4
            self.offsets[n] = (off, p.numel(), tuple(p.shape))
            off += p.numel()
        self.n_live = (off + 3) // 4 * 4
        off = self.n_live
        for n, p in dead:
            off = (off + 3) // 4 * 4
            self.offsets[n] = (off, p.numel(), tuple(p.shape))
            off += p.numel()
        self.n_total = (off + 3) // 4 * 4
        big0 = self.offsets["depth_projection.weight"][0] if "depth_projection.weight" in self.offsets else self.n_live
        self.bucket_small = (0, big0)
        self.bucket_big = (big0, self.n_live)
        self.params = torch.zeros(self.n_total, dtype=torch.float32, device=device)
        self.grads = torch.zeros(self.n_live, dtype=torch.float32, device=device)
        self.exp_avg = torch.zeros(self.n_live, dtype=torch.float32, device=device)
        self.exp_avg_sq = torch.zeros(self.n_live, dtype=torch.float32, device=device)
        self.live_names = [n for n, _ in live]
        with torch.no_grad():
            for n, p in named:
                o, k, shp = self.offsets[n]
                self.params[o:o + k].copy_(p.detach().reshape(-1).to(device=device, dtype=torch.float32))
                p.data = self.params[o:o + k].view(shp)
                p.grad = None

    def p(self, name):
        o, k, shp = self.offsets[name]
        return self.params[o:o + k].view(shp)

    def g(self, name):
        o, k, shp = self.offsets[name]
        return self.grads[o:o + k].view(shp)

    def attach_grads(self, named_params):
        for n, p in named_params:
            p.grad = self.g(n) if self.is_live(n) else None


class _Shape:

    def __init__(self, eng, B, S, train):
        dev, H, Q, K, L, heads = eng.device, eng.H, eng.Q, eng.K, eng.L, eng.heads
        N, BQ = B * S, B * Q
        f = lambda *s: torch.empty(*s, dtype=torch.float32, device=dev)
        self.B, self.S, self.N, self.BQ = B, S, N, BQ
        self.rgb, self.dep, self.dep_pre = f(N, H), f(N, H), f(N, H)
        self.mean_d, self.rstd_d = f(N), f(N)
        if eng.bn:
            self.bn_mean, self.bn_rstd, self.bn_absg = f(2, H), f(2, H), f(2, H)
            self.bn_idx = torch.empty(2, max(1, int(H * 0.1)), dtype=torch.int64, device=dev)
        self.sums = torch.empty(2, H, dtype=torch.float64, device=dev)
        self.idx = torch.empty(2, H // 4, dtype=torch.int64, device=dev)
        self.mask = f(2, H)
        self.x0, self.h1, self.vsw, self.x1, self.h2 = f(2 * N, H), f(2 * N, H), f(2 * N, H), f(2 * N, H), f(2 * N, H)
        self.u, self.f1 = f(2 * N, 4 * H), f(2 * N, 4 * H)
        self.x3, self.y = f(2 * N, H), f(2 * N, H)
        self.m1, self.r1, self.m2, self.r2, self.mf, self.rf = f(2 * N), f(2 * N), f(2 * N), f(2 * N), f(2 * N), f(2 * N)
        self.fused = f(N, H)
        self.tgt0 = torch.zeros(BQ, H, dtype=torch.float32, device=dev)
        self.layers = []
        for _ in range(L):
            d = dict(sa_qkv=f(BQ, 3 * H), sa_o=f(BQ, H), p_sa=f(B, heads, Q, Q), t1_pre=f(BQ, H),
                     t1=f(BQ, H), m1=f(BQ), r1=f(BQ), caq=f(BQ, H), cakv=f(N, 2 * H), ca_o=f(BQ, H),
                     p_ca=f(B, heads, Q, S), t2_pre=f(BQ, H), t2=f(BQ, H), m2=f(BQ), r2=f(BQ), ff1=f(BQ, 4 * H),
                     t3_pre=f(BQ, H), t3=f(BQ, H), m3=f(BQ), r3=f(BQ))
            self.layers.append(d)
        self.tgtF, self.mF, self.rF = f(BQ, H), f(BQ), f(BQ)
        self.actdur = f(BQ, K + 1)
        self.seg = f(N, K)
        self.loss = f(4)
        self.tables = {}
        self.loss_ws = torch.zeros(ops.losses_ws_floats(B, S, eng.Q), dtype=torch.float32, device=dev)
        self.counts = torch.zeros(4, dtype=torch.int64, device=dev)
        if train:
            self.d_actdur, self.d_seg = torch.zeros(BQ, K + 1, dtype=torch.float32, device=dev), f(N, K)
            self.d_tgtF, self.d_t = f(BQ, H), f(BQ, H)
            self.glayers = [dict(t3pre=f(BQ, H), ff2=f(BQ, H), ff1=f(BQ, 4 * H), t2=f(BQ, H), t2pre=f(BQ, H), cap=f(BQ, H),
                                 cao=f(BQ, H), caq=f(BQ, H), cakv=f(N, 2 * H), caqin=f(BQ, H), t1pre=f(BQ, H), sap=f(BQ, H),
                                 sao=f(BQ, H), saqkv=f(BQ, 3 * H), sain=f(BQ, H), t2b=f(BQ, H)) for _ in range(L)]
            self.d_fused, self.d_fused2 = f(N, H), f(N, H)
            lnw = lambda rows: f(max(ops.layernorm_bwd_ws_floats(rows, H), 4))
            self.lnp = dict(final=lnw(BQ), nf=lnw(2 * N), n2=lnw(2 * N), n1=lnw(2 * N), dep=lnw(N))
            self.lnp_seam = dict(n1=f(2 * N * H), dep=f(2 * N * H))
            for l in range(L):
                self.lnp.update({f"d3_{l}": lnw(BQ), f"d2_{l}": lnw(BQ), f"d1_{l}": lnw(BQ)})
            self.d_x3, self.d_u, self.d_h1, self.d_h2, self.d_x1, self.d_v, self.d_x0 = (
                f(2 * N, H), f(2 * N, 4 * H), f(2 * N, H), f(2 * N, H), f(2 * N, H), f(2 * N, H), f(2 * N, H))
            self.d_rgb_pre, self.d_dep, self.d_dep_pre = f(N, H), f(N, H), f(N, H)
            self.d_h2b = f(2 * N, H)
            if eng.bn:
                self.bn_terms = [f(N, H) for _ in range(5)]
            sizes = dict(x0=2 * N * H)
            for l in range(L):
                sizes.update({f"sa_p{l}": B * heads * Q * Q, f"ca_p{l}": B * heads * Q * S, f"d1_{l}": BQ * H,
                              f"d2_{l}": BQ * H, f"d3_{l}": BQ * H, f"ff_{l}": BQ * 4 * H})
            tot = sum((v + 15) // 16 * 16 for v in sizes.values())
            self.drop_pool = torch.ones(tot, dtype=torch.uint8, device=dev)
            self.drop, o = {}, 0
            for k, v in sizes.items():
                self.drop[k] = self.drop_pool[o:o + v]
                o += (v + 15) // 16 * 16


class FusionEngine:
    def __init__(self, module, device):
        self.module = module
        self.device = torch.device(device)
        assert self.device.type == "cuda", "the HIP engine needs an MI355X device (there is no CPU path)"
        ops._lib.load()
        self.H, self.Q, self.K = module.hidden_dim, module.n_query, module.n_class
        self.heads, self.L = module.n_head, module.num_decoder_layers
        self.dh = self.H // self.heads
        self.pad_idx = module.src_pad_idx
        self.P, self.D = module.depth_projection.in_features, module.input_embed.in_features
        assert self.H % 8 == 0 and self.H % self.heads == 0
        self.bn = hasattr(module.fuser, "bn_rgb")
        self.arena = ParamArena(list(module.named_parameters()), self.device, BN_LIVE_PREFIXES if self.bn else ())
        self.ws = ops.GemmWorkspace(self.device)
        self._sel = {}
        self.ws_side = ops.GemmWorkspace(self.device)
        self.side = torch.cuda.Stream(self.device)
        self.side2 = torch.cuda.Stream(self.device)
        self.ws_side2 = ops.GemmWorkspace(self.device)
        self.auto_side_stream = True
        self.use_side_stream = False
        self.use_fused_decoder = False
        self.use_fused_tail = True
        self.defer_tail = False
        self.use_paired_launches = True
        self.use_gemm_ln = True
        self.use_fuser_chain = True
        self.use_decoder_chain = True
        self.chain_bf3 = True
        self._planes = None
        self.overlap_planes = False
        self.overlap_param_tail = False
        self.ride_planes = True
        self._planes_rode = False
        self.fuse_depth_adamw = True
        self.pair_embeddings = True
        self._planes_forked = False
        self._tail_pending = False
        self._overlap_tail_now = False
        self.defer_loss_reduce = False
        self.loss_acc = None
        self.fold_rowsums = True
        self.ride_attention = True
        self.ride_attention_bwd = False
        self.split_k4h = False
        self.depth_prec = 1
        self.use_fused_embed = not self.bn
        self.dropout_enabled = bool(getattr(module, "r3d_dropout_enabled", True))
        self.erank_weight = 0.0
        self.erank_warm_start = False
        self.erank_max_sweeps = 16
        self.erank_side_stream = True
        self.er_stream = torch.cuda.Stream(self.device)
        self.ws_er = ops.GemmWorkspace(self.device)
        self._er_pending = False
        self.shapes = {}
        self.train_mask = None
        self.drop_seed = 0x5EED
        self.drop_offset = torch.zeros(1, dtype=torch.int64, device=self.device)
        self.lr_t = torch.zeros(1, dtype=torch.float32, device=self.device)
        self.step_t = torch.zeros(1, dtype=torch.int64, device=self.device)
        self._lr_host = None
        self.dur_den = None
        self.score_allreduce = None
        self.bn_sync = None
        self.grad_hook = None
        self.tp = None
        self._fw = None
        self.last = None
        self._adam = None
        self._drop_ready = None
        self.pos_grad_rows = 0
        a = self.arena
        K, H = self.K, self.H
        o_w = a.offsets["fc.weight"][0]
        self.w_head = a.params[o_w:o_w + (K + 1) * H].view(K + 1, H)
        self.gw_head = a.grads[o_w:o_w + (K + 1) * H].view(K + 1, H)
        o_b = a.offsets["fc.bias"][0]
        assert a.offsets["fc_len.weight"][0] == o_w + K * H and a.offsets["fc_len.bias"][0] == o_b + K
        self.b_head = a.params[o_b:o_b + K + 1]
        self.gb_head = a.grads[o_b:o_b + K + 1]

    def _shape(self, B, S, train):
        key = (B, S, bool(train))
        if key not in self.shapes:
            self.shapes[key] = _Shape(self, B, S, train)
        return self.shapes[key]

    def _train_masks(self, B, S):
        if self.train_mask is None:
            C = self.H
            sc = torch.full((2, C), 1.0 / (B * S * C), dtype=torch.float32, device=self.device)
            idx = torch.empty(2, C // 4, dtype=torch.int64, device=self.device)
            mask = torch.empty(2, C, dtype=torch.float32, device=self.device)
            ops.token_select(C // 4, idx, mask, score_f=sc)
            self.train_mask = (idx, mask)
        return self.train_mask

    def forward(self, feats, depth, labels, mode="train", training=False, need_grad=True, bn_training=None):
        self.forward_begin(feats, depth, labels, mode, training, need_grad)
        self._fw["bn_training"] = training if bn_training is None else bn_training
        if self._fw["tp"] is not None:
            self._fw["tp"].exchange_forward(self._fw["w"])
        return self.forward_finish()

    def forward_begin(self, feats, depth, labels, mode="train", training=False, need_grad=True):
        a, H = self.arena, self.H
        B, S = feats.shape[0], feats.shape[1]
        N = B * S
        assert feats.is_cuda and depth.is_cuda and feats.dtype == torch.float32 and depth.dtype == torch.float32
        x_rgb = feats.reshape(N, -1)
        x_dep = depth.reshape(N, -1)
        assert x_rgb.shape[1] == self.D and x_dep.shape[1] == self.P, (x_rgb.shape, x_dep.shape, self.D, self.P)
        assert x_rgb.is_contiguous() and x_dep.is_contiguous()
        w = self._shape(B, S, need_grad)
        self._loss_pending = None
        self._erank_join()
        drop = training and need_grad and self.dropout_enabled
        if drop:
            if self._drop_ready is w:
                self._drop_ready = None
            else:
                ops.dropout_mask(w.drop_pool, DROP_P, self.drop_seed, self.drop_offset)
        tp = self.tp if (self.tp is not None and need_grad) else None
        seam = self.use_fused_embed and mode == "train" and H <= 1024
        self._join_tail()
        if (self.overlap_planes and self.chain_bf3 and self.L == 1 and (self.use_fuser_chain or self.use_decoder_chain) and
                self._chain_shape_ok(w)):
            self.side.wait_stream(torch.cuda.current_stream())
            with torch.cuda.stream(self.side):
                self.chain_planes().refresh()
            self._planes_forked = True
        rgb_done = None
        dr = d = None
        if seam and tp is None and self.depth_prec == 1 and self.pair_embeddings:
            pr = ops.gemm_bf3_nt_pair(x_dep, a.p("depth_projection.weight"), w.dep_pre, self.ws,
                                      x_rgb, a.p("input_embed.weight"), w.rgb, self.ws_side)
            if pr is not None:
                d, dr = pr
        if dr is None:
            dr = ops.gemm(GEMM_NT, x_rgb, a.p("input_embed.weight"), w.rgb, bias=a.p("input_embed.bias"), act=1,
                          ws=self.ws_side if seam else self.ws, defer_reduce=seam, prec=self.depth_prec)
        slabs_r = self.ws_side.buf if (seam and dr.splitk > 1) else None
        if d is not None:
            pass
        elif tp is None:
            d = ops.gemm(GEMM_NT, x_dep, a.p("depth_projection.weight"), w.dep_pre, bias=a.p("depth_projection.bias"),
                         ws=self.ws, defer_reduce=True, prec=self.depth_prec)
        else:
            tp.partial_forward(w, x_dep, self.ws)
        slabs = self.ws.buf if (d is not None and d.splitk > 1) else None
        self._fw = dict(w=w, x_rgb=x_rgb, x_dep=x_dep, labels=labels, mode=mode, drop=drop, d=d, tp=tp, B=B, S=S,
                        slabs=slabs, seam=seam, dr=dr, slabs_r=slabs_r, rgb_done=rgb_done)

    def forward_finish(self):
        fw = self._fw
        w, x_rgb, x_dep, labels, mode, drop, d, tp = (fw[k] for k in ("w", "x_rgb", "x_dep", "labels", "mode", "drop", "d",
                                                                       "tp"))
        B, S = fw["B"], fw["S"]
        a, H, Q, K, heads, dh = self.arena, self.H, self.Q, self.K, self.heads, self.dh
        N, BQ = B * S, B * Q
        dsc = 1.0 / (1.0 - DROP_P)
        dm = (lambda k: w.drop[k]) if drop else (lambda k: None)
        key_labels = None
        if mode == "train":
            assert labels.dtype == torch.int64 and labels.is_cuda and labels.is_contiguous()
            key_labels = labels
        main = torch.cuda.current_stream()
        multi = self._multi_stream()
        s2 = self.side2 if multi else main
        ws2 = self.ws_side2 if multi else self.ws
        qpos = a.p("query_embed.weight")
        pos = a.p("pos_embedding")[0, :S]

        def sa_block(l, tgt_in, wsx):
            c, pl = w.layers[l], f"transformer.decoder.layers.{l}."
            ops.gemm(GEMM_NT, tgt_in, a.p(pl + "self_attn.in_proj_weight"), c["sa_qkv"], a_add=qpos, a_add_mod=Q,
                     bias=a.p(pl + "self_attn.in_proj_bias"), ws=wsx)
            ops.mha_core_fwd(c["sa_qkv"][:, :H], c["sa_qkv"][:, H:2 * H], c["sa_qkv"][:, 2 * H:], c["p_sa"], c["sa_o"], B,
                             heads, Q, Q, dh, drop_mask=dm(f"sa_p{l}"), drop_scale=dsc)
            if self._gln(BQ, H):
# ... 108 lines not shown
        if not paired:
            self._erank_fork(w)
        if paired:
            pass
        elif not fused_dec:
            if not hasattr(w, "fwd_group"):
                wi0 = a.p("transformer.decoder.layers.0.multihead_attn.in_proj_weight")
                bi0 = a.p("transformer.decoder.layers.0.multihead_attn.in_proj_bias")
                w.fwd_group = ops.GemmGroup(GEMM_NT, [
                    dict(a=w.fused, b=a.p("fc_seg.weight"), c=w.seg, bias=a.p("fc_seg.bias")),
                    dict(a=w.fused, b=wi0[H:], c=w.layers[0]["cakv"], bias=bi0[H:], a_add=pos, a_add_mod=S)],
                    tile=1 if H < 256 else 2)
            w.fwd_group.launch()
        else:
            ops.gemm(GEMM_NT, w.fused, a.p("fc_seg.weight"), w.seg, bias=a.p("fc_seg.bias"), ws=self.ws)
        self.last_drop_flag = bool(drop)
        if fused_dec:
            self._decoder_fused(w, key_labels, drop, dsc)
        else:
            self._decoder_unfused(w, key_labels, dm, dsc, multi, main, s2, sa_block, paired)
        if self._planes_forked:
            main.wait_stream(self.side)
            self._planes_forked = False
        self._planes_rode = False
        er = self.erank_weight != 0.0 and hasattr(w, "glayers")
        if er and not w.__dict__.get("_er_forked", False):
            self._erank_forward(w)
        w._er_forked = False
        self.last = dict(w=w, x_rgb=x_rgb, x_dep=x_dep, mask=mask, idx=idx, drop=drop, mode=mode, tp=tp, seam=seam, erank=er,
                         paired=paired, bn_training=bool(fw.get("bn_training", False)))
        return dict(seg=w.seg.view(B, S, K), action=w.actdur[:, :K].view(B, Q, K), duration=w.actdur[:, K].view(B, Q))

    def _erank_fork(self, w):
        if self.erank_weight == 0.0 or not hasattr(w, "glayers") or not self.erank_side_stream:
            return
        self.er_stream.wait_stream(torch.cuda.current_stream())
        with torch.cuda.stream(self.er_stream):
            self._erank_forward(w)
        w._er_forked = True
        self._er_pending = True

    def _erank_join(self):
        if self._er_pending:
            torch.cuda.current_stream().wait_stream(self.er_stream)
            self._er_pending = False

    def _erank_forward(self, w):
        N, H = w.N, self.H
        if not hasattr(w, "er_sigma"):
            f = lambda *s: torch.empty(*s, dtype=torch.float32, device=self.device)
            w.er_gout = f(1)
            w.er_blk = None
            if ops.erank_fits(N, H):
                w.er_sigma, w.er_stats, w.er_af = f(1, H), f(1, 4), f(1, H, N)
                w.er_vt = torch.eye(H, dtype=torch.float32, device=self.device)
                w.er_vraw, w.er_vg, w.er_gv, w.er_xw = f(H, H), f(H, H), f(H, H), f(N, H)
            else:
                w.er_flip = N < H
                R, Cc = (H, N) if w.er_flip else (N, H)
                w.er_blk = ops.ErankBlockedBufs(R, Cc, self.device, max_sweeps=self.erank_max_sweeps)
                w.er_sigma, w.er_stats = w.er_blk.sigma.view(1, Cc), w.er_blk.stats.view(1, 4)
        if w.er_blk is not None:
            ops.erank_blocked_into(w.fused, w.er_blk, transposed=w.er_flip)
        elif self.erank_warm_start and ops.erank_fits_warm(N, H):
            wsx = self.ws_er
            ops.gemm(GEMM_NT, w.fused, w.er_vt, w.er_xw, ws=wsx)
            ops.erank_jacobi_warm(w.er_xw, w.er_sigma, w.er_stats, w.er_vraw, vt_in=w.er_vt, af_t=w.er_af)
            ops.gemm(GEMM_NT, w.er_vraw, w.er_vraw, w.er_vg, ws=wsx)
            ops.gemm(GEMM_NN, w.er_vg, w.er_vraw, w.er_gv, ws=wsx)
            ops.erank_vt_polish(w.er_vraw, w.er_gv, w.er_vt)
        else:
            ops.erank_jacobi(w.fused, w.er_sigma, w.er_stats, af_t=w.er_af)

    def _erank_backward(self, w, ws, dst=None):
        from .erank import ErankBackward
        if not hasattr(w, "er_bwd"):
            w.er_bwd = ErankBackward(w.N, self.H, w.er_blk is not None and w.er_flip, self.device)
        w.er_gout.fill_(-float(self.erank_weight))
        A = w.er_blk.af_t if w.er_blk is not None else w.er_af[0]
        w.er_bwd.run(w.fused, A, w.er_sigma[0], w.er_stats[0], w.er_gout, dst if dst is not None else w.d_fused2,
                     dst is None, ws)

    def erank_value(self):
        self._erank_join()
        return self.last["w"].er_stats[0, 0]

    def chain_planes(self):
        if self._planes is None:
            a, H = self.arena, self.H
            pre, pl = "fuser.blocks.0.", "transformer.decoder.layers.0."
            wi = a.p(pl + "multihead_attn.in_proj_weight")
            W = dict(wv=a.p(pre + "attn.qkv.weight")[2 * H:], wproj=a.p(pre + "attn.proj.weight"), w1=a.p(pre + "mlp.mlp.0.weight"),
                     w2=a.p(pre + "mlp.mlp.2.weight"), wkv=wi[H:], wseg=a.p("fc_seg.weight"),
                     dec_wo=a.p(pl + "multihead_attn.out_proj.weight"), dec_w1=a.p(pl + "linear1.weight"),
                     dec_w2=a.p(pl + "linear2.weight"))
            ent = {}
            for k, w_ in W.items():
                ent["pl_" + k] = (w_, False)
                ent["pl_" + k + "_t"] = (w_, True)
            self._planes = ops.WeightPlanes(ent, self.device)
        return self._planes

    def _multi_stream(self):
        return bool(self.use_side_stream or (self.auto_side_stream and self.H >= 512 and self.tp is None and
                                             self.grad_hook is None))

    def _planes_refresh(self):
        if self._planes_forked:
            torch.cuda.current_stream().wait_stream(self.side)
            self._planes_forked = False
        elif self._planes_rode:
            pass
        else:
            self.chain_planes().refresh()

    def _join_tail(self):
        if self._tail_pending:
            torch.cuda.current_stream().wait_stream(self.side)
            self._tail_pending = False

    def _chain_shape_ok(self, w):
        return fuser_chain_shape_ok(w.B, w.S, self.H, self.K, self.Q, self.heads, self.bn)

    def _chain_ok(self, w):
        return bool(self.use_fuser_chain and self._chain_shape_ok(w))

    def _dec_chain_ok(self, w):
        return bool(self.use_decoder_chain and decoder_chain_shape_ok(w.B, w.S, self.H, self.Q, self.heads, self.L))

    def _dec_chain(self, w, drop):
        bf3 = bool(self.chain_bf3)
        key = ("dec_chain", bool(drop), bf3)
        if bf3 and not (self.use_fuser_chain and self._chain_shape_ok(w)):
            self._planes_refresh()
        if key not in w.tables:
            pls = self.chain_planes() if bf3 else None
            dpl = None
            if pls is not None:
                dpl = dict(pl_wo=pls.ptr("pl_dec_wo"), pl_w1=pls.ptr("pl_dec_w1"), pl_w2=pls.ptr("pl_dec_w2"),
                           pl_w2_t=pls.ptr("pl_dec_w2_t"), pl_w1_t=pls.ptr("pl_dec_w1_t"), pl_wo_t=pls.ptr("pl_dec_wo_t"))
            a, H = self.arena, self.H
            c, pl = w.layers[0], "transformer.decoder.layers.0."
            dk = (lambda k: w.drop[k]) if drop else (lambda k: None)
            gl = w.glayers[0] if hasattr(w, "glayers") else None
            g = (lambda k: gl[k]) if gl is not None else (lambda k: None)
            w.tables[key] = ops.DecoderChain(
                caq=c["caq"], cakv=c["cakv"], p_ca=c["p_ca"], drop_ca=dk("ca_p0"), ca_o=c["ca_o"],
                wo=a.p(pl + "multihead_attn.out_proj.weight"), bo=a.p(pl + "multihead_attn.out_proj.bias"), drop_d2=dk("d2_0"),
                t1=c["t1"], t2_pre=c["t2_pre"], g2=a.p(pl + "norm2.weight"), be2=a.p(pl + "norm2.bias"), t2=c["t2"], m2=c["m2"],
                r2=c["r2"], w1=a.p(pl + "linear1.weight"), b1=a.p(pl + "linear1.bias"), drop_ff=dk("ff_0"), ff1=c["ff1"],
                w2=a.p(pl + "linear2.weight"), b2=a.p(pl + "linear2.bias"), drop_d3=dk("d3_0"), t3_pre=c["t3_pre"],
                d_t3pre=g("t3pre"), d_ff2=g("ff2"), d_ff1=g("ff1"), d_t2pre=g("t2pre"), d_cap=g("cap"), d_cao=g("cao"),
                d_caq=g("caq"), d_cakv=g("cakv"), part_d2=w.lnp["d2_0"] if gl is not None else None,
                drop_scale=1.0 / (1.0 - DROP_P), pad_idx=self.pad_idx, B=w.B, S=w.S, H=H, Q=self.Q, heads=self.heads, planes=dpl)
        return w.tables[key]

    def _gln(self, rows, K):
        return self.use_gemm_ln and ops.gemm_ln_supported(rows, K, self.H)

    def _forward_paired(self, w, fw, dm, dsc, drop, wv, pre, qpos, pos):
        a, H, Q, S, B, BQ, heads, dh = self.arena, self.H, self.Q, w.S, w.B, w.BQ, self.heads, self.dh
        c, pl = w.layers[0], "transformer.decoder.layers.0."
        if self._chain_ok(w):
            bf3 = bool(self.chain_bf3)
            key = ("fwd_chain", bool(drop), bf3)
            if bf3:
                self._planes_refresh()
            if key not in w.tables:
                pls = self.chain_planes() if bf3 else None
                wi, bi = a.p(pl + "multihead_attn.in_proj_weight"), a.p(pl + "multihead_attn.in_proj_bias")
                w.tables[key] = ops.FuserChainFwd(
                    x0=w.x0, h1=w.h1, wv=wv, wproj=a.p(pre + "attn.proj.weight"), bproj=a.p(pre + "attn.proj.bias"),
                    g2=a.p(pre + "norm2.weight"), be2=a.p(pre + "norm2.bias"), w1=a.p(pre + "mlp.mlp.0.weight"),
                    b1=a.p(pre + "mlp.mlp.0.bias"), w2=a.p(pre + "mlp.mlp.2.weight"), b2=a.p(pre + "mlp.mlp.2.bias"),
                    gf=a.p("fuser.norm.weight"), bef=a.p("fuser.norm.bias"), pos=pos.contiguous(), wkv=wi[H:], bkv=bi[H:],
                    wseg=a.p("fc_seg.weight"), bseg=a.p("fc_seg.bias"), vsw=w.vsw, x1=w.x1, h2=w.h2, m2=w.m2, r2=w.r2, u=w.u,
                    f1=w.f1, x3=w.x3, y=w.y, mf=w.mf, rf=w.rf, fused=w.fused, seg=w.seg, cakv=c["cakv"],
                    qpos=qpos, w_in=a.p(pl + "self_attn.in_proj_weight"), b_in=a.p(pl + "self_attn.in_proj_bias"),
                    w_out=a.p(pl + "self_attn.out_proj.weight"), b_out=a.p(pl + "self_attn.out_proj.bias"),
                    g1=a.p(pl + "norm1.weight"), be1=a.p(pl + "norm1.bias"), wq=wi[:H], bq=bi[:H],
                    drop_sa=dm("sa_p0"), drop_d1=dm("d1_0"), drop_scale=dsc, sa_qkv=c["sa_qkv"], p_sa=c["p_sa"],
                    sa_o=c["sa_o"], t1_pre=c["t1_pre"], t1=c["t1"], m1=c["m1"], r1=c["r1"], caq=c["caq"],
                    N=w.N, S=S, K=self.K, H=H, add_xres=0 if self.bn else 1, B=B, Q=Q, heads=heads,
                    planes={k: pls.ptr(k) for k in pls.keys if not k.endswith("_t") and "dec_" not in k} if pls is not None else None)
            w.tables[key].launch()
            self._erank_fork(w)
            return
        key = ("fwd_pairs", bool(drop))
        if key not in w.tables:
            wi, bi = a.p(pl + "multihead_attn.in_proj_weight"), a.p(pl + "multihead_attn.in_proj_bias")
            t = 1 if H < 256 else 2
            g1 = ops.GemmGroup(GEMM_NT, [
                dict(a=w.h1, b=wv, c=w.vsw, c_row_xor=1),
                dict(a=w.tgt0, b=a.p(pl + "self_attn.in_proj_weight"), c=c["sa_qkv"], a_add=qpos, a_add_mod=Q,
                     bias=a.p(pl + "self_attn.in_proj_bias"))], tile=t)
            g2 = ops.GemmGroup(GEMM_NT, [
                dict(a=w.h2, b=a.p(pre + "mlp.mlp.0.weight"), c=w.f1, bias=a.p(pre + "mlp.mlp.0.bias"), act=2, pre_out=w.u),
                dict(a=c["sa_o"], b=a.p(pl + "self_attn.out_proj.weight"), c=c["t1_pre"],
                     bias=a.p(pl + "self_attn.out_proj.bias"), drop_mask=self._dm2(dm("d1_0"), BQ, H), drop_scale=dsc)],
                tile=t)
            g3 = ops.GemmGroup(GEMM_NT, [
                dict(a=w.fused, b=a.p("fc_seg.weight"), c=w.seg, bias=a.p("fc_seg.bias")),
                dict(a=w.fused, b=wi[H:], c=c["cakv"], bias=bi[H:], a_add=pos, a_add_mod=S),
                dict(a=c["t1"], b=wi[:H], c=c["caq"], a_add=qpos, a_add_mod=Q, bias=bi[:H])], tile=t)
            w.tables[key] = (g1, g2, g3)
        g1, g2, g3 = w.tables[key]
        g1.launch()
        gln = self._gln(2 * w.N, H) and self._gln(2 * w.N, 4 * H) and self._gln(BQ, 0)
        sa = dict(q=c["sa_qkv"][:, :H], k=c["sa_qkv"][:, H:2 * H], v=c["sa_qkv"][:, 2 * H:], probs=c["p_sa"], o=c["sa_o"], B=B,
                  heads=heads, Lq=Q, Lk=Q, dh=dh, drop_mask=dm("sa_p0"), drop_scale=dsc)
        ride = gln and self.ride_attention and ops.gemm_ln_mha_supported(heads, Q, Q, dh)
        if gln:
            ops.gemm_ln_fwd([dict(a=w.vsw, w=a.p(pre + "attn.proj.weight"), bias=a.p(pre + "attn.proj.bias"), res1=w.x0,
                                  pre=w.x1, gamma=a.p(pre + "norm2.weight"), beta=a.p(pre + "norm2.bias"), y=w.h2,
                                  mean=w.m2, rstd=w.r2)], mha=sa if ride else None)
        else:
            ops.gemm(GEMM_NT, w.vsw, a.p(pre + "attn.proj.weight"), w.x1, bias=a.p(pre + "attn.proj.bias"), res1=w.x0,
                     ws=self.ws)
        if not ride:
            ops.mha_core_fwd(sa["q"], sa["k"], sa["v"], sa["probs"], sa["o"], B, heads, Q, Q, dh, drop_mask=sa["drop_mask"],
                             drop_scale=dsc)
        if not gln:
            ops.layernorm_fwd(w.x1, a.p(pre + "norm2.weight"), a.p(pre + "norm2.bias"), w.h2, w.m2, w.r2)
        g2.launch()
        if gln:
            ops.gemm_ln_fwd([
                dict(a=w.f1, w=a.p(pre + "mlp.mlp.2.weight"), bias=a.p(pre + "mlp.mlp.2.bias"), res1=w.x1,
                     res2=None if self.bn else w.x0, pre=w.x3, gamma=a.p("fuser.norm.weight"),
                     beta=a.p("fuser.norm.bias"), y=w.y, mean=w.mf, rstd=w.rf, pair_out=w.fused),
                dict(a=None, pre=c["t1_pre"], gamma=a.p(pl + "norm1.weight"), beta=a.p(pl + "norm1.bias"), y=c["t1"],
                     mean=c["m1"], rstd=c["r1"])])
        else:
            ops.gemm(GEMM_NT, w.f1, a.p(pre + "mlp.mlp.2.weight"), w.x3, bias=a.p(pre + "mlp.mlp.2.bias"), res1=w.x1,
                     res2=None if self.bn else w.x0, ws=self.ws)
            ops.layernorm_fwd_multi([
                dict(x=c["t1_pre"], gamma=a.p(pl + "norm1.weight"), beta=a.p(pl + "norm1.bias"), y=c["t1"], mean=c["m1"],
                     rstd=c["r1"]),
                dict(x=w.x3, gamma=a.p("fuser.norm.weight"), beta=a.p("fuser.norm.bias"), y=w.y, mean=w.mf, rstd=w.rf,
                     pair_out=w.fused)])
        self._erank_fork(w)
        g3.launch()

    def _decoder_unfused(self, w, key_labels, dm, dsc, multi, main, s2, sa_block, paired=False):
        a, H, Q, K, heads, dh = self.arena, self.H, self.Q, self.K, self.heads, self.dh
        B, S, N, BQ = w.B, w.S, w.N, w.BQ
        pos = a.p("pos_embedding")[0, :S]
        tgt = None
        for l in range(self.L):
            c, pl = w.layers[l], f"transformer.decoder.layers.{l}."
            wi, bi = a.p(pl + "multihead_attn.in_proj_weight"), a.p(pl + "multihead_attn.in_proj_bias")
            if l > 0:
                ops.gemm(GEMM_NT, w.fused, wi[H:], c["cakv"], a_add=pos, a_add_mod=S, bias=bi[H:], ws=self.ws)
            if l == 0:
                if multi:
                    main.wait_stream(s2)
            else:
                sa_block(l, tgt, self.ws)
            w._dec_deferred = False
            if paired and self._dec_chain_ok(w):
                drop_now = self.last_drop_flag
                w._tail_done = False
                w._tail_deferred = bool(self.use_fused_tail and self.defer_tail and self._fw["mode"] == "train" and
                                        hasattr(w, "glayers") and tail_in_decoder_chain(B, H, self.K, Q))
                w._dec_key_labels = key_labels
                if w._tail_deferred:
                    w._dec_deferred = True
                    return
                self._dec_chain(w, drop_now).launch(1, key_label=key_labels)
                if self.use_fused_tail:
                    ops.decoder_tail_fwd(c["t3_pre"], a.p(pl + "norm3.weight"), a.p(pl + "norm3.bias"),
                                         a.p("transformer.decoder.norm.weight"), a.p("transformer.decoder.norm.bias"),
                                         self.w_head, self.b_head, c["t3"], c["m3"], c["r3"], w.tgtF, w.mF, w.rF, w.actdur)
                    return
                ops.layernorm_fwd(c["t3_pre"], a.p(pl + "norm3.weight"), a.p(pl + "norm3.bias"), c["t3"], c["m3"], c["r3"])
                tgt = c["t3"]
                continue
            ops.mha_core_fwd(c["caq"], c["cakv"][:, :H], c["cakv"][:, H:], c["p_ca"], c["ca_o"], B, heads, Q, S, dh,
                             key_labels=key_labels, pad_idx=self.pad_idx, drop_mask=dm(f"ca_p{l}"), drop_scale=dsc)
            if self._gln(BQ, H):
                ops.gemm_ln_fwd([dict(a=c["ca_o"], w=a.p(pl + "multihead_attn.out_proj.weight"),
                                      bias=a.p(pl + "multihead_attn.out_proj.bias"),
                                      drop_mask=self._dm2(dm(f"d2_{l}"), BQ, H), drop_scale=dsc, res1=c["t1"],
                                      pre=c["t2_pre"], gamma=a.p(pl + "norm2.weight"), beta=a.p(pl + "norm2.bias"),
                                      y=c["t2"], mean=c["m2"], rstd=c["r2"])])
            else:
                ops.gemm(GEMM_NT, c["ca_o"], a.p(pl + "multihead_attn.out_proj.weight"), c["t2_pre"],
                         bias=a.p(pl + "multihead_attn.out_proj.bias"), drop_mask=self._dm2(dm(f"d2_{l}"), BQ, H),
                         drop_scale=dsc, res1=c["t1"], ws=self.ws)
                ops.layernorm_fwd(c["t2_pre"], a.p(pl + "norm2.weight"), a.p(pl + "norm2.bias"), c["t2"], c["m2"], c["r2"])
            ops.gemm(GEMM_NT, c["t2"], a.p(pl + "linear1.weight"), c["ff1"], bias=a.p(pl + "linear1.bias"), act=1,
                     drop_mask=self._dm2(dm(f"ff_{l}"), BQ, 4 * H), drop_scale=dsc, ws=self.ws)
            ops.gemm(GEMM_NT, c["ff1"], a.p(pl + "linear2.weight"), c["t3_pre"], bias=a.p(pl + "linear2.bias"),
                     drop_mask=self._dm2(dm(f"d3_{l}"), BQ, H), drop_scale=dsc, res1=c["t2"], ws=self.ws)
            if l == self.L - 1 and self.use_fused_tail:
                w._tail_done = False
                w._tail_deferred = bool(self.defer_tail and self._fw["mode"] == "train" and hasattr(w, "glayers")
                                        and tail_in_decoder_chain(B, H, self.K, Q))
                if w._tail_deferred:
                    return
                ops.decoder_tail_fwd(c["t3_pre"], a.p(pl + "norm3.weight"), a.p(pl + "norm3.bias"),
                                     a.p("transformer.decoder.norm.weight"), a.p("transformer.decoder.norm.bias"),
                                     self.w_head, self.b_head, c["t3"], c["m3"], c["r3"], w.tgtF, w.mF, w.rF, w.actdur)
                return
            ops.layernorm_fwd(c["t3_pre"], a.p(pl + "norm3.weight"), a.p(pl + "norm3.bias"), c["t3"], c["m3"], c["r3"])
            tgt = c["t3"]
        ops.layernorm_fwd(tgt, a.p("transformer.decoder.norm.weight"), a.p("transformer.decoder.norm.bias"), w.tgtF,
                          w.mF, w.rF)
# ... 598 lines not shown
```

### r3d_amd/ops.py

```python
import ctypes as C

import torch

from . import _lib
from ._lib import GemmDesc, GEMM_NT, GEMM_NN, GEMM_TN, check


def _stream():
    return C.c_void_p(torch.cuda.current_stream().cuda_stream)


def _pv(t):
    return None if t is None else t.data_ptr()


def _p(t):
    if t is None:
        return None
    assert t.is_cuda, "r3d_amd kernels take device tensors only"
    return C.c_void_p(t.data_ptr())


def _f32(t, name="tensor"):
    assert t.dtype == torch.float32 and t.is_cuda, f"{name} must be a float32 device tensor"
# ... 262 lines not shown


def gemm_ln_supported(M, K, H):
    return bool(_lib.load().r3d_gemm_ln_supported(int(M), int(K), int(H)))


def gemm_ln_mha_supported(heads, Lq, Lk, dh):
    return bool(_lib.load().r3d_gemm_ln_mha_supported(int(heads), int(Lq), int(Lk), int(dh)))


def gemm_ln_fwd(jobs, mha=None):
    from ._lib import GemmLnJob
    arr = (GemmLnJob * len(jobs))()
    H = jobs[0]["pre"].shape[1]
    for i, j in enumerate(jobs):
        g = lambda k: j.get(k)
        a, t = arr[i], g("a")
        M = j["pre"].shape[0]
        assert j["pre"].shape[1] == H
        if t is not None:
            _f32(t, "A"), _f32(j["w"], "W")
            assert j["w"].shape == (H, t.shape[1]) and t.shape[0] == M
            a.A, a.lda, a.W, a.ldw, a.K = t.data_ptr(), _ld(t), j["w"].data_ptr(), _ld(j["w"]), t.shape[1]
            a.bias = _pv(g("bias"))
            a.drop_mask, a.lddrop = _pv(g("drop_mask")), _ld(g("drop_mask")) if g("drop_mask") is not None else 0
            a.drop_scale = g("drop_scale") or 1.0
            a.res1, a.ldr1 = _pv(g("res1")), _ld(g("res1")) if g("res1") is not None else 0
            a.res2, a.ldr2 = _pv(g("res2")), _ld(g("res2")) if g("res2") is not None else 0
        else:
            a.K = 0
        a.pre_out, a.ldpre = j["pre"].data_ptr(), _ld(j["pre"])
        a.gamma, a.beta, a.y, a.ldy = j["gamma"].data_ptr(), j["beta"].data_ptr(), j["y"].data_ptr(), _ld(j["y"])
        a.mean, a.rstd = j["mean"].data_ptr(), j["rstd"].data_ptr()
        a.pair_out = _pv(g("pair_out"))
        a.M = M
    if mha is not None:
        from ._lib import MhaJob
        m, g = MhaJob(), mha.get
        m.q, m.ldq, m.k, m.ldk, m.v, m.ldv = (mha["q"].data_ptr(), _ld(mha["q"]), mha["k"].data_ptr(), _ld(mha["k"]),
                                              mha["v"].data_ptr(), _ld(mha["v"]))
        m.key_padding_mask, m.key_label, m.pad_idx = _pv(g("kpm")), _pv(g("key_labels")), g("pad_idx") or 0
        m.probs, m.drop_mask, m.drop_scale = mha["probs"].data_ptr(), _pv(g("drop_mask")), g("drop_scale") or 1.0
        m.o, m.ldo = mha["o"].data_ptr(), _ld(mha["o"])
        m.B, m.heads, m.Lq, m.Lk, m.dh = mha["B"], mha["heads"], mha["Lq"], mha["Lk"], mha["dh"]
        check(_lib.load().r3d_gemm_ln_mha_fwd(arr, len(jobs), H, C.byref(m), _stream()), "r3d_gemm_ln_mha_fwd")
        return
    check(_lib.load().r3d_gemm_ln_fwd(arr, len(jobs), H, _stream()), "r3d_gemm_ln_fwd")


def fuser_chain_supported(N, H, K, B, Q, heads):
    return bool(_lib.load().r3d_fuser_chain_supported(N, H, K, B, Q, heads))


class WeightPlanes:

    def __init__(self, entries, device):
        from ._lib import PlaneJob
        lib = _lib.load()
        self.keys = list(entries)
        sizes, offs, total_el, blocks = [], [], 0, 0
        jobs = (PlaneJob * len(self.keys))()
        for i, k in enumerate(self.keys):
            w, tr = entries[k]
            assert w.dim() == 2 and w.stride(1) == 1 and w.dtype == torch.float32 and w.is_cuda
            N, K = (w.shape[1], w.shape[0]) if tr else (w.shape[0], w.shape[1])
            el = int(lib.r3d_weight_plane_elems(N, K))
            offs.append(total_el)
            sizes.append((N, K))
            j = jobs[i]
            j.src, j.ld, j.N, j.K, j.transposed, j.first_block = w.data_ptr(), w.stride(0), N, K, 1 if tr else 0, blocks
            total_el += el
            blocks += ((N + 15) // 16) * ((K + 31) // 32)
        self.buf = torch.zeros(total_el, dtype=torch.int16, device=device)
        for i in range(len(self.keys)):
            jobs[i].dst = self.buf.data_ptr() + 2 * offs[i]
        raw = bytes(jobs)
        self.jobs_dev = torch.frombuffer(bytearray(raw), dtype=torch.uint8).to(device)
        self.njobs, self.blocks = len(self.keys), blocks
        self._ptr = {k: self.buf.data_ptr() + 2 * offs[i] for i, k in enumerate(self.keys)}
        self._view = {k: self.buf[offs[i]:offs[i] + int(lib.r3d_weight_plane_elems(*sizes[i]))] for i, k in enumerate(self.keys)}

    def refresh(self):
        check(_lib.load().r3d_weight_planes(_p(self.jobs_dev), self.njobs, self.blocks, _stream()), "r3d_weight_planes")

    def ptr(self, key):
        return self._ptr[key]

    def view(self, key):
        return self._view[key]


class FuserChainFwd:

    def __init__(self, **t):
        from ._lib import FuserChainFwdArgs
        a = FuserChainFwdArgs()
        dims = {k: t.pop(k) for k in ("N", "S", "K", "H", "add_xres", "B", "Q", "heads")}
        a.drop_scale = float(t.pop("drop_scale", 1.0))
        opt = {"y", "drop_sa", "drop_d1"}
        planes = t.pop("planes", None)
        if planes is not None:
            for name in FuserChainFwdArgs._PLANES:
                setattr(a, name, planes[name])
        for name in FuserChainFwdArgs._PTRS + FuserChainFwdArgs._PTRS2:
            v = t.pop(name, None)
            if v is None:
                assert name in opt, name
                continue
            assert v.is_cuda and v.is_contiguous(), name
            assert v.dtype == (torch.uint8 if name.startswith("drop_") else torch.float32), name
            setattr(a, name, v.data_ptr())
        assert not t, t.keys()
        for k, v in dims.items():
            setattr(a, k, int(v))
        self.args = a

    def launch(self):
        check(_lib.load().r3d_fuser_chain_fwd(C.byref(self.args), _stream()), "r3d_fuser_chain_fwd")


class FuserChainBwd:

    def __init__(self, **t):
        from ._lib import FuserChainBwdArgs
        a = FuserChainBwdArgs()
        dims = {k: t.pop(k) for k in ("N", "S", "K", "H", "add_xres", "B", "Q", "heads")}
        a.drop_scale = float(t.pop("drop_scale", 1.0))
        opt = {"d_extra", "drop_x0", "drop_d1", "drop_sa", "d_h2", "d_h1", "t1pre_out"}
        planes = t.pop("planes", None)
        if planes is not None:
            for name in FuserChainBwdArgs._PLANES:
                setattr(a, name, planes[name])
        for name in FuserChainBwdArgs._PTRS:
            v = t.pop(name, None)
            if v is None:
                assert name in opt, name
                continue
            assert v.is_cuda and v.is_contiguous(), name
            assert v.dtype == (torch.uint8 if name.startswith("drop_") else torch.float32), name
            setattr(a, name, v.data_ptr())
        assert not t, t.keys()
        for k, v in dims.items():
            setattr(a, k, int(v))
        self.args = a

    def launch(self):
        check(_lib.load().r3d_fuser_chain_bwd(C.byref(self.args), _stream()), "r3d_fuser_chain_bwd")


def decoder_chain_supported(H, Q, heads, S):
    return bool(_lib.load().r3d_decoder_chain_supported(H, Q, heads, S))


class DecoderChain:

    def __init__(self, **t):
        from ._lib import DecoderChainArgs
        a = DecoderChainArgs()
        dims = {k: t.pop(k) for k in ("pad_idx", "B", "S", "H", "Q", "heads")}
        a.drop_scale = float(t.pop("drop_scale", 1.0))
        opt = {"key_label", "drop_ca", "drop_d2", "drop_ff", "drop_d3", "d_t3pre", "d_ff2", "d_ff1", "d_t2pre", "d_cap", "d_cao",
               "d_caq", "d_cakv", "part_d2"}
        planes = t.pop("planes", None)
        if planes is not None:
            for name in ("pl_wo", "pl_w1", "pl_w2", "pl_w2_t", "pl_w1_t", "pl_wo_t"):
                setattr(a, name, planes[name])
        for name in DecoderChainArgs._PTRS:
            v = t.pop(name, None)
            if v is None:
                assert name in opt, name
                continue
            assert v.is_cuda and v.is_contiguous(), name
            want = torch.uint8 if name.startswith("drop_") else (torch.int64 if name == "key_label" else torch.float32)
            assert v.dtype == want, name
            setattr(a, name, v.data_ptr())
        assert not t, t.keys()
        for k, v in dims.items():
            setattr(a, k, int(v))
        self.args = a

    def launch(self, phases, key_label=None, tail=None, ws=None):
        a = self.args
        a.phases = int(phases)
        a.key_label = None if key_label is None else key_label.data_ptr()
        check(_lib.load().r3d_decoder_chain(C.byref(a), C.byref(tail) if tail is not None else None, _p(ws), _stream()),
              "r3d_decoder_chain")


def layernorm_bwd_multi(jobs, mha=None):
    from ._lib import LnBwdJob
    arr = (LnBwdJob * len(jobs))()
    for i, j in enumerate(jobs):
        rows, H = j["x"].shape
        a = arr[i]
        g = lambda k: j.get(k)
        a.dy, a.lddy, a.pair_in = j["dy"].data_ptr(), _ld(j["dy"]), 1 if g("pair_in") else 0
        a.dy2, a.lddy2 = _pv(g("dy2")), _ld(g("dy2")) if g("dy2") is not None else 0
        a.x, a.ldx, a.mean, a.rstd = j["x"].data_ptr(), _ld(j["x"]), j["mean"].data_ptr(), j["rstd"].data_ptr()
        a.gamma, a.beta, a.relu = j["gamma"].data_ptr(), j["beta"].data_ptr(), 1 if g("relu") else 0
        a.add1, a.ldadd1 = _pv(g("add1")), _ld(g("add1")) if g("add1") is not None else 0
        a.add2, a.ldadd2 = _pv(g("add2")), _ld(g("add2")) if g("add2") is not None else 0
        a.dx, a.lddx = j["dx"].data_ptr(), _ld(j["dx"])
        a.dx2, a.lddx2 = _pv(g("dx2")), _ld(g("dx2")) if g("dx2") is not None else 0
        a.drop_mask, a.lddrop = _pv(g("drop_mask")), _ld(g("drop_mask")) if g("drop_mask") is not None else 0
        a.drop_scale = g("drop_scale") or 1.0
        a.dgamma, a.dbeta, a.ws = j["dgamma"].data_ptr(), j["dbeta"].data_ptr(), j["partial"].data_ptr()
        a.rows, a.H = rows, H
        assert j["partial"].numel() >= _lib.load().r3d_layernorm_bwd_ws_floats(rows, H)
    if mha is not None:
        from ._lib import MhaBwdJob
        m, gg = MhaBwdJob(), mha.get
        for n in ("q", "k", "v"):
            setattr(m, n, mha[n].data_ptr())
            setattr(m, "ld" + n, _ld(mha[n]))
        m.probs, m.drop_mask, m.drop_scale = mha["probs"].data_ptr(), _pv(gg("drop_mask")), gg("drop_scale") or 1.0
        m.d_o, m.lddo = mha["d_o"].data_ptr(), _ld(mha["d_o"])
        for n in ("dq", "dk", "dv"):
            setattr(m, n, mha[n].data_ptr())
            setattr(m, "ld" + n, _ld(mha[n]))
        m.B, m.heads, m.Lq, m.Lk, m.dh = mha["B"], mha["heads"], mha["Lq"], mha["Lk"], mha["dh"]
        check(_lib.load().r3d_layernorm_bwd_multi_mha(arr, len(jobs), C.byref(m), _stream()), "r3d_layernorm_bwd_multi_mha")
        return
    check(_lib.load().r3d_layernorm_bwd_multi(arr, len(jobs), _stream()), "r3d_layernorm_bwd_multi")


def layernorm_bwd_finalize(partial, rows, H, dgamma, dbeta):
    lib = _lib.load()
    check(lib.r3d_layernorm_bwd_finalize(_p(partial), rows, H, _p(dgamma), _p(dbeta), _stream()), "r3d_layernorm_bwd_finalize")


def layernorm_bwd_ws_floats(rows, H):
    return int(_lib.load().r3d_layernorm_bwd_ws_floats(rows, H))


def add_rowbcast(x, add, mod, out):
    lib = _lib.load()
    rows, cols = out.shape
    check(lib.r3d_add_rowbcast(_p(x), _ld(x) if x is not None else 0, _p(add), _ld(add), mod, _p(out), _ld(out), rows, cols,
                               _stream()), "r3d_add_rowbcast")


def colsum(x, out, *, accumulate=False, ws=None):
    lib = _lib.load()
    rows, cols = x.shape
    need = lib.r3d_colsum_ws_floats(rows, cols)
    wsb = ws.get(need) if need > 0 else None
    check(lib.r3d_colsum(_p(x), _ld(x), rows, cols, _p(out), _p(wsb), 1 if accumulate else 0, _stream()), "r3d_colsum")


def rowmod_sum(x, mod, out, *, accumulate=False):
    lib = _lib.load()
    rows, cols = x.shape
    check(lib.r3d_rowmod_sum(_p(x), _ld(x), rows, cols, mod, _p(out), _ld(out), 1 if accumulate else 0, _stream()),
          "r3d_rowmod_sum")


def colabssum(x, out):
    lib = _lib.load()
    rows, cols = x.shape
    assert out.dtype == torch.float64
    check(lib.r3d_colabssum(_p(x), _ld(x), rows, cols, _p(out), _stream()), "r3d_colabssum")


def token_select(k, idx_out, mask_out, *, score_f=None, score_sum=None, count=0.0, used_serial=None):
    lib = _lib.load()
    src = score_f if score_f is not None else score_sum
    nvec, Cc = src.shape
    assert src.is_contiguous() and idx_out.dtype == torch.int64 and tuple(idx_out.shape) == (nvec, k)
    check(lib.r3d_token_select(_p(score_f), _p(score_sum), float(count), nvec, Cc, k, _p(idx_out), _p(mask_out),
                               _p(used_serial), _stream()), "r3d_token_select")


def token_exchange_fwd(rgb, dep, mask_rgb, mask_dep, x0, *, drop_mask=None, drop_scale=1.0):
    lib = _lib.load()
    N, H = rgb.shape
    assert rgb.is_contiguous() and dep.is_contiguous() and x0.is_contiguous()
    check(lib.r3d_token_exchange_fwd(_p(rgb), _p(dep), _p(mask_rgb), _p(mask_dep), _p(x0), _p(drop_mask), drop_scale, N, H,
                                     _stream()), "r3d_token_exchange_fwd")


def token_exchange_bwd(dx0, rgb, mask_rgb, mask_dep, d_rgb_pre, d_dep, *, drop_mask=None, drop_scale=1.0):
    lib = _lib.load()
    N, H = rgb.shape
    check(lib.r3d_token_exchange_bwd(_p(dx0), _p(rgb), _p(mask_rgb), _p(mask_dep), _p(drop_mask), drop_scale, _p(d_rgb_pre),
                                     _p(d_dep), N, H, _stream()), "r3d_token_exchange_bwd")


def mha_core_fwd(q, k, v, probs, o, B, heads, Lq, Lk, dh, *, kpm=None, key_labels=None, pad_idx=0, drop_mask=None,
                 drop_scale=1.0):
    lib = _lib.load()
    check(lib.r3d_mha_core_fwd(_p(q), _ld(q), _p(k), _ld(k), _p(v), _ld(v), _p(kpm), _p(key_labels), pad_idx, _p(probs), _p(drop_mask),
                               drop_scale, _p(o), _ld(o), B, heads, Lq, Lk, dh, _stream()), "r3d_mha_core_fwd")


def mha_core_bwd(q, k, v, probs, d_o, dq, dk, dv, B, heads, Lq, Lk, dh, *, drop_mask=None, drop_scale=1.0):
    lib = _lib.load()
    check(lib.r3d_mha_core_bwd(_p(q), _ld(q), _p(k), _ld(k), _p(v), _ld(v), _p(probs), _p(drop_mask), drop_scale, _p(d_o),
                               _ld(d_o), _p(dq), _ld(dq), _p(dk), _ld(dk), _p(dv), _ld(dv), B, heads, Lq, Lk, dh,
                               _stream()), "r3d_mha_core_bwd")


def decoder_fused_supported(S, Q, H, heads):
    return bool(_lib.load().r3d_decoder_fused_supported(S, Q, H, heads))


class PtrTable:

    def __init__(self, tensors):
        self._keep = tensors
        self.n = len(tensors)
        self.arr = (C.c_void_p * self.n)(*[(t.data_ptr() if t is not None else None) for t in tensors])


def decoder_layer_fwd(table, B, S, Q, H, heads, pad_idx, drop_scale, n_head_out):
    check(_lib.load().r3d_decoder_layer_fwd(table.arr, table.n, B, S, Q, H, heads, pad_idx, drop_scale, n_head_out, _stream()),
          "r3d_decoder_layer_fwd")


def bn_stats(x_rgb, x_dep, bn_rgb, bn_dep, mean, rstd, absg, training, momentum=0.1):
    N, Cc = x_rgb.shape
    check(_lib.load().r3d_bn_stats(_p(x_rgb), _p(x_dep), _p(bn_rgb.running_mean), _p(bn_rgb.running_var),
                                   _p(bn_rgb.num_batches_tracked), _p(bn_dep.running_mean), _p(bn_dep.running_var),
                                   _p(bn_dep.num_batches_tracked), _p(bn_rgb.weight), _p(bn_dep.weight), _p(mean), _p(rstd),
                                   _p(absg), N, Cc, 1 if training else 0, momentum, _stream()), "r3d_bn_stats")


def bn_blend_fwd(rgb, dep, mean, rstd, g_r, b_r, g_d, b_d, alpha, m_rgb, m_dep, drop, drop_scale, ln1_g, ln1_b, x0, h1, m1, r1):
    N, Cc = rgb.shape
    check(_lib.load().r3d_bn_blend_fwd(_p(rgb), _p(dep), _p(mean), _p(rstd), _p(g_r), _p(b_r), _p(g_d), _p(b_d), _p(alpha),
                                       _p(m_rgb), _p(m_dep), _p(drop), drop_scale, _p(ln1_g), _p(ln1_b), _p(x0), _p(h1),
                                       _p(m1), _p(r1), N, Cc, _stream()), "r3d_bn_blend_fwd")


def bn_blend_bwd(d_h1, x0, m1, r1, ln1_g, add1, drop, drop_scale, rgb, dep, mean, rstd, g_r, b_r, g_d, b_d, alpha, m_rgb, m_dep,
                 t0, t1, t2, t3, t4, ws_n1):
    N, Cc = rgb.shape
    assert ws_n1.numel() >= 2 * N * Cc
# ... 363 lines not shown
```

Baseline: 44380.

## Split each decoder-chain clip across a group of cooperating blocks

The bf3 decoder chain kernel now spreads each clip over G blocks (G of 1, 2 or 4, picked from batch size), and each block computes a slice of the FFN columns. Blocks swap intermediate FFN activations, t3 partial results and tail gradients through a global-memory workspace, synchronised by spin-waiting on atomic counters with a timeout. The aim is to fill more compute units when the batch is small, since one block per clip leaves the GPU underused. In exchange it adds inter-block global traffic, spin synchronisation that depends on all group blocks being resident at once, a larger workspace and an ABI change.

```diff
diff --git a/include/r3d_hip.h b/include/r3d_hip.h
--- a/include/r3d_hip.h
+++ b/include/r3d_hip.h
@@ -7,7 +7,7 @@
 extern "C" {
 #endif
 
-#define R3D_ABI_VERSION 2
+#define R3D_ABI_VERSION 3
 
 #define R3D_OK 0
 #define R3D_EINVAL (-1)
@@ -283,8 +283,10 @@
     uint64_t* timeline;
     const uint16_t* pl_wo; const uint16_t* pl_w1; const uint16_t* pl_w2; const uint16_t* pl_w2_t; const uint16_t* pl_w1_t;
     const uint16_t* pl_wo_t;
+    int32_t group;
 } r3d_decoder_chain_args;
 int r3d_decoder_chain_supported(int H, int Q, int heads, int S);
+int r3d_decoder_chain_ws_layout(int B, int S, int Q, int group, int64_t* out);
 int r3d_decoder_chain(const r3d_decoder_chain_args* d, const r3d_tail_losses_args* tail, float* ws, void* stream);
 
 int r3d_adamw_flat(float* p, const float* g, float* m, float* v, int64_t n, const float* lr, const int64_t* step,
diff --git a/r3d_amd/_lib.py b/r3d_amd/_lib.py
--- a/r3d_amd/_lib.py
+++ b/r3d_amd/_lib.py
@@ -3,7 +3,7 @@
 
 HERE = os.path.dirname(os.path.abspath(__file__))
 LIB_PATH = os.path.join(HERE, "_build", "libr3d_hip.so")
-ABI_VERSION = 2
+ABI_VERSION = 3
 
 c_float_p = C.c_void_p
 
@@ -91,7 +91,7 @@
              "t3_pre d_t3pre d_ff2 d_ff1 d_t2pre d_cap d_cao d_caq d_cakv part_d2").split()
     _fields_ = ([(n, C.c_void_p) for n in _PTRS] + [("drop_scale", C.c_float)] +
                 [(n, C.c_int32) for n in "pad_idx B S H Q heads phases".split()] + [("timeline", C.c_void_p)] +
-                [(n, C.c_void_p) for n in "pl_wo pl_w1 pl_w2 pl_w2_t pl_w1_t pl_wo_t".split()])
+                [(n, C.c_void_p) for n in "pl_wo pl_w1 pl_w2 pl_w2_t pl_w1_t pl_wo_t".split()] + [("group", C.c_int32)])
 
 
 class MhaJob(C.Structure):
@@ -174,6 +174,7 @@
     "r3d_triple_mean_bwd": ([_P, _P, _I, _I, _P], C.c_int),
     "r3d_decoder_chain_supported": ([_I, _I, _I, _I], C.c_int),
     "r3d_decoder_chain": ([_P, _P, _P, _P], C.c_int),
+    "r3d_decoder_chain_ws_layout": ([_I, _I, _I, _I, _P], C.c_int),
     "r3d_gemm_ln_mha_supported": ([_I, _I, _I, _I], C.c_int),
     "r3d_gemm_ln_mha_fwd": ([_P, _I, _I, _P, _P], C.c_int),
     "r3d_layernorm_fwd_multi": ([_P, _I, _P], C.c_int),
diff --git a/r3d_amd/csrc/decoder_chain.hip b/r3d_amd/csrc/decoder_chain.hip
--- a/r3d_amd/csrc/decoder_chain.hip
+++ b/r3d_amd/csrc/decoder_chain.hip
@@ -299,7 +299,105 @@
     bf3_store4(img, kD3P1, r, 4 * c4, r < 8 ? v : z);
 }
 
-__device__ __forceinline__ void dc3_fwd(const DcArgs& D, const int b, float* lds) {
+enum { kDxFf1 = 0, kDxT3 = 1, kDxTail = 2, kDxDff1 = 3, kDxD = 4, kDxDone = 5 };
+constexpr int kDxSlotFf1 = 0;
+constexpr int kDxSlotT3 = kDxSlotFf1 + 8 * 4 * kFcH;
+constexpr int kDxSlotRes = kDxSlotT3 + 8 * kFcH;
+constexpr int kDxSlotDff2 = kDxSlotRes + 8 * kFcH;
+constexpr int kDxSlotDff1 = kDxSlotDff2 + 8 * kFcH;
+constexpr int kDxSlotD = kDxSlotDff1 + 8 * 4 * kFcH;
+constexpr int kDxClipFloats = kDxSlotD + 8 * kFcH;
+constexpr int kDxCtrLine = 32;
+constexpr unsigned long long kDxSpinTicks = 2000000ull;
+constexpr int kDxSc1 = 16;
+typedef unsigned u32x4 __attribute__((ext_vector_type(4)));
+
+struct DcX {
+    float* slots;
+    unsigned* ctr;
+    unsigned* err;
+    int* fail;
+};
+
+__device__ __forceinline__ __amdgpu_buffer_rsrc_t dx_rsrc(const DcX& x) {
+    return __builtin_amdgcn_make_buffer_rsrc(x.slots, (short)0, kDxClipFloats * 4, 0x00020000);
+}
+__device__ __forceinline__ void dx_put(const DcX& x, int base, int c, int q, const f32x4 v) {
+    if (q < 2)
+        __builtin_amdgcn_raw_buffer_store_b128(__builtin_bit_cast(u32x4, v), dx_rsrc(x), (base + c * 8 + 4 * q) * 4, 0, kDxSc1);
+}
+__device__ __forceinline__ f32x4 dx_get(const DcX& x, int base, int c, int q) {
+    const f32x4 v = __builtin_bit_cast(
+        f32x4, __builtin_amdgcn_raw_buffer_load_b128(dx_rsrc(x), (base + c * 8 + 4 * (q & 1)) * 4, 0, kDxSc1));
+    const f32x4 z = {0.f, 0.f, 0.f, 0.f};
+    return q < 2 ? v : z;
+}
+__device__ __forceinline__ void dx_arrive(const DcX& x, int k) {
+    asm volatile("s_waitcnt vmcnt(0)" ::: "memory");
+    __syncthreads();
+    if (threadIdx.x == 0) __hip_atomic_fetch_add(x.ctr + k, 1u, __ATOMIC_RELAXED, __HIP_MEMORY_SCOPE_AGENT);
+}
+__device__ __forceinline__ void dx_wait(const DcX& x, int k, unsigned target) {
+    if (threadIdx.x == 0 && !*x.fail) {
+        const unsigned long long t0 = wall_clock64();
+        while (__hip_atomic_load(x.ctr + k, __ATOMIC_RELAXED, __HIP_MEMORY_SCOPE_AGENT) < target) {
+            if (wall_clock64() - t0 > kDxSpinTicks) {
+                __hip_atomic_fetch_or(x.err, 1u << k, __ATOMIC_RELAXED, __HIP_MEMORY_SCOPE_AGENT);
+                *x.fail = 1;
+                break;
+            }
+            __builtin_amdgcn_s_sleep(2);
+        }
+    }
+    __syncthreads();
+}
+__device__ __forceinline__ void dx_finish(const DcX& x, int G) {
+    __syncthreads();
+    if (threadIdx.x == 0 &&
+        __hip_atomic_fetch_add(x.ctr + kDxDone, 1u, __ATOMIC_RELAXED, __HIP_MEMORY_SCOPE_AGENT) == (unsigned)(G - 1)) {
+        for (int k = 0; k <= kDxDone; ++k) __hip_atomic_store(x.ctr + k, 0u, __ATOMIC_RELAXED, __HIP_MEMORY_SCOPE_AGENT);
+    }
+}
+template <int G>
+__device__ __forceinline__ void dx_gather_ffn(const DcX& x, int base, unsigned short* imgF, int m, int wave, int li, int q) {
+    constexpr int T = 4 / G;
+#pragma unroll
+    for (int mm = 0; mm < G; ++mm) {
+        if (mm == m) continue;
+#pragma unroll
+        for (int t = 0; t < T; ++t) {
+            const int cu = ((32 / G) * mm + T * wave + t) * 16 + li;
+            const f32x4 v = dx_get(x, base, cu, q);
+#pragma unroll
+            for (int i = 0; i < 4; ++i) bf3_store1(imgF, kD3P4, 4 * q + i, cu, v[i]);
+        }
+    }
+}
+
+template <int G>
+struct Dc3Keep {
+    float ffv[4 / G][4], t2p[4], mean[4], rstd[4];
+    uint8_t kbf[4 / G][4], kb2[4];
+};
+
+template <int G>
+__device__ __forceinline__ void dc3_fwd_load(Bf3B& r, const DcArgs& D, int j, int m, int wave, int lane) {
+    constexpr int T = 4 / G;
+    if (j == 0) bf3_bload<4>(r, D.pl_wo, 4, wave, 0, lane);
+    else if (j <= T) bf3_bload<4>(r, D.pl_w1, 4, (32 / G) * m + T * wave + (j - 1), 0, lane);
+    else bf3_bload<4>(r, D.pl_w2, 16, wave, 4 * (j - 1 - T), lane);
+}
+template <int G>
+__device__ __forceinline__ void dc3_bwd_load(Bf3B& r, const DcArgs& D, int j, int m, int wave, int lane) {
+    constexpr int T = 4 / G;
+    if (j < T) bf3_bload<4>(r, D.pl_w2_t, 4, (32 / G) * m + T * wave + j, 0, lane);
+    else if (j < T + 4) bf3_bload<4>(r, D.pl_w1_t, 16, wave, 4 * (j - T), lane);
+    else bf3_bload<4>(r, D.pl_wo_t, 4, wave, 0, lane);
+}
+
+template <int G>
+__device__ __forceinline__ void dc3_fwd(const DcArgs& D, const int b, const int m, float* lds, const DcX& x, Dc3Keep<G>& kp) {
+    constexpr int T = 4 / G;
     const int tid = threadIdx.x, lane = tid & 63, wave = tid >> 6;
     const int li = lane & 15, q = lane >> 4;
     unsigned short* img = reinterpret_cast<unsigned short*>(lds);
@@ -312,105 +410,187 @@
     const int row0 = b * 8;
     const int c = wave * 16 + li;
     const bool live = q < 2;
+    const bool own = G == 1 || (wave * G) / 8 == m;
+    const int nc = own ? 5 + T : 1 + T;
+    const bool mk = b == 0 && m == 0;
     const f32x4 zero = {0.f, 0.f, 0.f, 0.f};
-    R3D_CHAIN_MARK(D.timeline, b == 0, 0);
-    Bf3B b0, b1, b2;
-    bf3_bload<4>(b0, D.pl_wo, 4, wave, 0, lane);
-    bf3_bload<4>(b1, D.pl_w1, 4, 4 * wave + 0, 0, lane);
-    bf3_bload<4>(b2, D.pl_w1, 4, 4 * wave + 1, 0, lane);
+    R3D_CHAIN_MARK(D.timeline, mk, 0);
+    Bf3B bb[3];
+#pragma unroll
+    for (int j = 0; j < 3; ++j)
+        if (j < nc) dc3_fwd_load<G>(bb[j], D, j, m, wave, lane);
     const FcMaskSrc md2(D.drop_d2, D.g2, H), md3(D.drop_d3, D.g2, H), mff(D.drop_ff, D.g2, 4 * H);
     float t1v[4];
-    uint8_t kb2[4], kb3[4], kbf[4][4];
+    uint8_t kb3[4];
 #pragma unroll
     for (int i = 0; i < 4; ++i) {
         const size_t r = (size_t)(row0 + ((4 * q + i) & 7));
         t1v[i] = D.t1[r * H + c];
-        kb2[i] = md2.raw(r, c);
+        kp.kb2[i] = md2.raw(r, c);
         kb3[i] = md3.raw(r, c);
 #pragma unroll
-        for (int t = 0; t < 4; ++t) kbf[t][i] = mff.raw(r, (4 * wave + t) * 16 + li);
+        for (int t = 0; t < T; ++t) kp.kbf[t][i] = mff.raw(r, ((32 / G) * m + T * wave + t) * 16 + li);
     }
     const float b_o = D.bo[c], g2 = D.g2[c], be2 = D.be2[c], b_2 = D.b2[c];
-    float b_1[4];
-#pragma unroll
-    for (int t = 0; t < 4; ++t) b_1[t] = D.b1[(4 * wave + t) * 16 + li];
-    R3D_CHAIN_MARK(D.timeline, b == 0, 1);
+    float b_1[T];
+#pragma unroll
+    for (int t = 0; t < T; ++t) b_1[t] = D.b1[((32 / G) * m + T * wave + t) * 16 + li];
+    R3D_CHAIN_MARK(D.timeline, mk, 1);
     {
-        MhaArgs m{};
-        m.q = D.caq; m.ldq = H; m.k = D.cakv; m.ldk = 2 * H; m.v = D.cakv + H; m.ldv = 2 * H;
-        m.key_label = D.key_label; m.pad_idx = D.pad_idx; m.probs = D.p_ca; m.drop = D.drop_ca; m.drop_scale = D.drop_scale;
-        m.o = D.ca_o; m.ldo = H; m.B = D.B; m.heads = 8; m.Lq = 8; m.Lk = D.S; m.dh = 16; m.scale = 0.25f;
-        mha_fwd_small_unit<16, 8, false>(m, b * 8 + wave, scr);
-    }
-    R3D_CHAIN_MARK(D.timeline, b == 0, 2);
+        MhaArgs a{};
+        a.q = D.caq; a.ldq = H; a.k = D.cakv; a.ldk = 2 * H; a.v = D.cakv + H; a.ldv = 2 * H;
+        a.key_label = D.key_label; a.pad_idx = D.pad_idx; a.probs = D.p_ca; a.drop = D.drop_ca; a.drop_scale = D.drop_scale;
+        a.o = D.ca_o; a.ldo = H; a.B = D.B; a.heads = 8; a.Lq = 8; a.Lk = D.S; a.dh = 16; a.scale = 0.25f;
+        mha_fwd_small_unit<16, 8, false>(a, b * 8 + wave, scr);
+    }
+    R3D_CHAIN_MARK(D.timeline, mk, 2);
     __syncthreads();
     dc3_stage_rows(imgA, D.ca_o, row0, tid);
     __syncthreads();
-    R3D_CHAIN_MARK(D.timeline, b == 0, 3);
+    R3D_CHAIN_MARK(D.timeline, mk, 3);
     f32x4 acc0 = zero, acc1 = zero;
-    bf3_chunk<4>(imgA, kD3P1, li, q, 0, b0, acc0, acc1);
-    __builtin_amdgcn_sched_barrier(0);
-    bf3_bload<4>(b0, D.pl_w1, 4, 4 * wave + 2, 0, lane);
-    __builtin_amdgcn_sched_barrier(0);
-    float t2p[4], mean[4], rstd[4], t2v[4];
+    bf3_chunk<4>(imgA, kD3P1, li, q, 0, bb[0], acc0, acc1);
+    __builtin_amdgcn_sched_barrier(0);
+    if (3 < nc) dc3_fwd_load<G>(bb[0], D, 3, m, wave, lane);
+    __builtin_amdgcn_sched_barrier(0);
+    float mean[4], rstd[4], t2v[4];
 #pragma unroll
     for (int i = 0; i < 4; ++i) {
-        t2p[i] = ((acc0[i] + acc1[i]) + b_o) * md2.keep(kb2[i], D.drop_scale) + t1v[i];
-        if (live) D.t2_pre[(size_t)(row0 + 4 * q + i) * H + c] = t2p[i];
-    }
-    fc_layernorm(t2p, red, wave, li, q, mean, rstd);
+        kp.t2p[i] = ((acc0[i] + acc1[i]) + b_o) * md2.keep(kp.kb2[i], D.drop_scale) + t1v[i];
+        if (live && own) D.t2_pre[(size_t)(row0 + 4 * q + i) * H + c] = kp.t2p[i];
+    }
+    fc_layernorm(kp.t2p, red, wave, li, q, mean, rstd);
 #pragma unroll
     for (int i = 0; i < 4; ++i) {
-        t2v[i] = (t2p[i] - mean[i]) * rstd[i] * g2 + be2;
+        kp.mean[i] = mean[i]; kp.rstd[i] = rstd[i];
+        t2v[i] = (kp.t2p[i] - mean[i]) * rstd[i] * g2 + be2;
         const int r = 4 * q + i;
-        if (live) {
+        if (live && own) {
             D.t2[(size_t)(row0 + r) * H + c] = t2v[i];
             if (wave == 0 && li == 0) { D.m2[row0 + r] = mean[i]; D.r2[row0 + r] = rstd[i]; }
         }
         bf3_store1(imgB, kD3P1, r, c, live ? t2v[i] : 0.f);
     }
     __syncthreads();
-    R3D_CHAIN_MARK(D.timeline, b == 0, 4);
-#pragma unroll
-    for (int t = 0; t < 4; ++t) {
+    R3D_CHAIN_MARK(D.timeline, mk, 4);
+#pragma unroll
+    for (int t = 0; t < T; ++t) {
+        const int j = 1 + t;
         acc0 = zero; acc1 = zero;
-        if (t == 0) bf3_chunk<4>(imgB, kD3P1, li, q, 0, b1, acc0, acc1);
-        if (t == 1) bf3_chunk<4>(imgB, kD3P1, li, q, 0, b2, acc0, acc1);
-        if (t == 2) bf3_chunk<4>(imgB, kD3P1, li, q, 0, b0, acc0, acc1);
-        if (t == 3) bf3_chunk<4>(imgB, kD3P1, li, q, 0, b1, acc0, acc1);
+        bf3_chunk<4>(imgB, kD3P1, li, q, 0, bb[j % 3], acc0, acc1);
         __builtin_amdgcn_sched_barrier(0);
-        if (t == 0) bf3_bload<4>(b1, D.pl_w1, 4, 4 * wave + 3, 0, lane);
-        if (t == 1) bf3_bload<4>(b2, D.pl_w2, 16, wave, 0, lane);
-        if (t == 2) bf3_bload<4>(b0, D.pl_w2, 16, wave, 4, lane);
-        if (t == 3) bf3_bload<4>(b1, D.pl_w2, 16, wave, 8, lane);
+        if (j + 3 < nc) dc3_fwd_load<G>(bb[j % 3], D, j + 3, m, wave, lane);
         __builtin_amdgcn_sched_barrier(0);
-        const int cu = (4 * wave + t) * 16 + li;
-#pragma unroll
-        for (int i = 0; i < 4; ++i) {
-            const float f = fmaxf((acc0[i] + acc1[i]) + b_1[t], 0.f) * mff.keep(kbf[t][i], D.drop_scale);
+        const int cu = ((32 / G) * m + T * wave + t) * 16 + li;
+        f32x4 fv;
+#pragma unroll
+        for (int i = 0; i < 4; ++i) {
+            const float f = fmaxf((acc0[i] + acc1[i]) + b_1[t], 0.f) * mff.keep(kp.kbf[t][i], D.drop_scale);
+            kp.ffv[t][i] = f;
+            fv[i] = f;
             if (live) D.ff1[(size_t)(row0 + 4 * q + i) * (4 * H) + cu] = f;
             bf3_store1(imgF, kD3P4, 4 * q + i, cu, live ? f : 0.f);
         }
-    }
-    __syncthreads();
-    R3D_CHAIN_MARK(D.timeline, b == 0, 5);
-    acc0 = zero; acc1 = zero;
-    bf3_chunk<4>(imgF, kD3P4, li, q, 0, b2, acc0, acc1);
-    __builtin_amdgcn_sched_barrier(0);
-    bf3_bload<4>(b2, D.pl_w2, 16, wave, 12, lane);
-    __builtin_amdgcn_sched_barrier(0);
-    bf3_chunk<4>(imgF, kD3P4, li, q, 4, b0, acc0, acc1);
-    bf3_chunk<4>(imgF, kD3P4, li, q, 8, b1, acc0, acc1);
-    bf3_chunk<4>(imgF, kD3P4, li, q, 12, b2, acc0, acc1);
+        if (G > 1) dx_put(x, kDxSlotFf1, cu, q, fv);
+    }
+    if (G > 1) {
+        R3D_CHAIN_MARK(D.timeline, mk, 16);
+        dx_arrive(x, kDxFf1);
+        dx_wait(x, kDxFf1, G);
+        R3D_CHAIN_MARK(D.timeline, mk, 17);
+        dx_gather_ffn<G>(x, kDxSlotFf1, imgF, m, wave, li, q);
+    }
+    __syncthreads();
+    R3D_CHAIN_MARK(D.timeline, mk, 5);
+    f32x4 t3 = zero;
+    if (own) {
+        acc0 = zero; acc1 = zero;
+#pragma unroll
+        for (int t = 0; t < 4; ++t) {
+            const int j = 1 + T + t;
+            bf3_chunk<4>(imgF, kD3P4, li, q, 4 * t, bb[j % 3], acc0, acc1);
+            __builtin_amdgcn_sched_barrier(0);
+            if (j + 3 < nc) dc3_fwd_load<G>(bb[j % 3], D, j + 3, m, wave, lane);
+            __builtin_amdgcn_sched_barrier(0);
+        }
+#pragma unroll
+        for (int i = 0; i < 4; ++i) t3[i] = ((acc0[i] + acc1[i]) + b_2) * md3.keep(kb3[i], D.drop_scale) + t2v[i];
+    }
+    if (G > 1) {
+        if (m != 0) {
+            if (own) dx_put(x, kDxSlotT3, c, q, t3);
+            dx_arrive(x, kDxT3);
+            return;
+        }
+        dx_wait(x, kDxT3, G - 1);
+        R3D_CHAIN_MARK(D.timeline, mk, 18);
+        if (!own) t3 = dx_get(x, kDxSlotT3, c, q);
+    }
     if (live) {
 #pragma unroll
-        for (int i = 0; i < 4; ++i)
-            D.t3_pre[(size_t)(row0 + 4 * q + i) * H + c] =
-                ((acc0[i] + acc1[i]) + b_2) * md3.keep(kb3[i], D.drop_scale) + t2v[i];
-    }
-}
-
-__device__ __forceinline__ void dc3_bwd(const DcArgs& D, const int b, float* lds) {
+        for (int i = 0; i < 4; ++i) D.t3_pre[(size_t)(row0 + 4 * q + i) * H + c] = t3[i];
+    }
+}
+
+__device__ __forceinline__ void dc3_publish_tail(const DcArgs& D, const int b, const DcX& x) {
+    const int lane = threadIdx.x & 63, wave = threadIdx.x >> 6, li = lane & 15, q = lane >> 4;
+    const int c = wave * 16 + li;
+    f32x4 r, f;
+#pragma unroll
+    for (int i = 0; i < 4; ++i) {
+        const size_t e = (size_t)(b * 8 + ((4 * q + i) & 7)) * kFcH + c;
+        r[i] = D.d_t3pre[e];
+        f[i] = D.d_ff2[e];
+    }
+    dx_put(x, kDxSlotRes, c, q, r);
+    dx_put(x, kDxSlotDff2, c, q, f);
+    dx_arrive(x, kDxTail);
+    R3D_CHAIN_MARK(D.timeline, b == 0, 19);
+}
+
+__device__ __forceinline__ void dc3_rowsum2(const float (&g)[4], const float (&xh)[4], float* red, int wave, int li, int q,
+                                            float (&sa)[4], float (&sb)[4]) {
+#pragma clang fp contract(off)
+#pragma unroll
+    for (int i = 0; i < 4; ++i) {
+        float a = g[i];
+        a += dpp_mov_f<0x128>(a);
+        a += dpp_mov_f<0x124>(a);
+        a += dpp_mov_f<0x122>(a);
+        a += dpp_mov_f<0x121>(a);
+        sa[i] = a;
+        const float x = g[i] * xh[i];
+        float y = __builtin_fmaf(g[i], xh[i], dpp_mov_f<0x128>(x));
+        y += dpp_mov_f<0x124>(y);
+        y += dpp_mov_f<0x122>(y);
+        y += dpp_mov_f<0x121>(y);
+        sb[i] = y;
+    }
+    if (li == 0) {
+#pragma unroll
+        for (int i = 0; i < 4; ++i) {
+            red[(0 * 8 + wave) * kFcRows + 4 * q + i] = sa[i];
+            red[(1 * 8 + wave) * kFcRows + 4 * q + i] = sb[i];
+        }
+    }
+    __syncthreads();
+#pragma unroll
+    for (int i = 0; i < 4; ++i) {
+        float x = 0.f, y = 0.f;
+#pragma unroll
+        for (int w8 = 0; w8 < 8; ++w8) {
+            x += red[(0 * 8 + w8) * kFcRows + 4 * q + i];
+            y += red[(1 * 8 + w8) * kFcRows + 4 * q + i];
+        }
+        sa[i] = x * (1.0f / (float)kFcH);
+        sb[i] = y * (1.0f / (float)kFcH);
+    }
+}
+
+template <int G>
+__device__ __forceinline__ void dc3_bwd(const DcArgs& D, const int b, const int m, float* lds, const DcX& x, Dc3Keep<G>& kp,
+                                        const bool fwd_here, const bool tail_here) {
+    constexpr int T = 4 / G;
     const int tid = threadIdx.x, lane = tid & 63, wave = tid >> 6;
     const int li = lane & 15, q = lane >> 4;
     unsigned short* img = reinterpret_cast<unsigned short*>(lds);
@@ -422,136 +602,193 @@
     const int row0 = b * 8;
     const int c = wave * 16 + li;
     const bool live = q < 2;
+    const bool own = G == 1 || (wave * G) / 8 == m;
+    const int nc = own ? T + 5 : T;
+    const bool mk = b == 0 && m == 0;
     const f32x4 zero = {0.f, 0.f, 0.f, 0.f};
-    R3D_CHAIN_MARK(D.timeline, b == 0, 10);
-    Bf3B b0, b1, b2;
-    bf3_bload<4>(b0, D.pl_w2_t, 4, 4 * wave + 0, 0, lane);
-    bf3_bload<4>(b1, D.pl_w2_t, 4, 4 * wave + 1, 0, lane);
-    bf3_bload<4>(b2, D.pl_w2_t, 4, 4 * wave + 2, 0, lane);
-    dc3_stage_rows(imgA, D.d_ff2, row0, tid);
+    R3D_CHAIN_MARK(D.timeline, mk, 10);
+    Bf3B bb[3];
+#pragma unroll
+    for (int j = 0; j < 3; ++j)
+        if (j < nc) dc3_bwd_load<G>(bb[j], D, j, m, wave, lane);
     const FcMaskSrc md2(D.drop_d2, D.g2, H), mff(D.drop_ff, D.g2, 4 * H);
-    float ffv[4][4], res[4], t2pv[4], m2v[4], r2v[4];
-    uint8_t kb2[4], kbf[4][4];
-#pragma unroll
-    for (int i = 0; i < 4; ++i) {
-        const size_t r = (size_t)(row0 + ((4 * q + i) & 7));
-#pragma unroll
-        for (int t = 0; t < 4; ++t) {
-            ffv[t][i] = D.ff1[r * (4 * H) + (4 * wave + t) * 16 + li];
-            kbf[t][i] = mff.raw(r, (4 * wave + t) * 16 + li);
-        }
-        res[i] = D.d_t3pre[r * H + c];
-        t2pv[i] = D.t2_pre[r * H + c];
-        m2v[i] = D.m2[r]; r2v[i] = D.r2[r];
-        kb2[i] = md2.raw(r, c);
-    }
+    if (!fwd_here) {
+#pragma unroll
+        for (int i = 0; i < 4; ++i) {
+            const size_t r = (size_t)(row0 + ((4 * q + i) & 7));
+#pragma unroll
+            for (int t = 0; t < T; ++t) {
+                const int cu = ((32 / G) * m + T * wave + t) * 16 + li;
+                kp.ffv[t][i] = D.ff1[r * (4 * H) + cu];
+                kp.kbf[t][i] = mff.raw(r, cu);
+            }
+            kp.t2p[i] = D.t2_pre[r * H + c];
+            kp.mean[i] = D.m2[r]; kp.rstd[i] = D.r2[r];
+            kp.kb2[i] = md2.raw(r, c);
+        }
+    }
+    f32x4 res, dff2;
+    if (G > 1 && m != 0 && tail_here) {
+        dx_wait(x, kDxTail, 1);
+        res = dx_get(x, kDxSlotRes, c, q);
+        dff2 = dx_get(x, kDxSlotDff2, c, q);
+    } else {
+#pragma unroll
+        for (int i = 0; i < 4; ++i) {
+            const size_t e = (size_t)(row0 + ((4 * q + i) & 7)) * H + c;
+            res[i] = D.d_t3pre[e];
+            dff2[i] = D.d_ff2[e];
+        }
+    }
+#pragma unroll
+    for (int i = 0; i < 4; ++i) bf3_store1(imgA, kD3P1, 4 * q + i, c, live ? dff2[i] : 0.f);
     const float g2 = D.g2[c];
     __syncthreads();
-    R3D_CHAIN_MARK(D.timeline, b == 0, 11);
+    R3D_CHAIN_MARK(D.timeline, mk, 11);
     f32x4 acc0, acc1;
 #pragma unroll
-    for (int t = 0; t < 4; ++t) {
+    for (int t = 0; t < T; ++t) {
         acc0 = zero; acc1 = zero;
-        if (t == 0) bf3_chunk<4>(imgA, kD3P1, li, q, 0, b0, acc0, acc1);
-        if (t == 1) bf3_chunk<4>(imgA, kD3P1, li, q, 0, b1, acc0, acc1);
-        if (t == 2) bf3_chunk<4>(imgA, kD3P1, li, q, 0, b2, acc0, acc1);
-        if (t == 3) bf3_chunk<4>(imgA, kD3P1, li, q, 0, b0, acc0, acc1);
+        bf3_chunk<4>(imgA, kD3P1, li, q, 0, bb[t % 3], acc0, acc1);
         __builtin_amdgcn_sched_barrier(0);
-        if (t == 0) bf3_bload<4>(b0, D.pl_w2_t, 4, 4 * wave + 3, 0, lane);
-        if (t == 1) bf3_bload<4>(b1, D.pl_w1_t, 16, wave, 0, lane);
-        if (t == 2) bf3_bload<4>(b2, D.pl_w1_t, 16, wave, 4, lane);
-        if (t == 3) bf3_bload<4>(b0, D.pl_w1_t, 16, wave, 8, lane);
+        if (t + 3 < nc) dc3_bwd_load<G>(bb[t % 3], D, t + 3, m, wave, lane);
         __builtin_amdgcn_sched_barrier(0);
-        const int cu = (4 * wave + t) * 16 + li;
-#pragma unroll
-        for (int i = 0; i < 4; ++i) {
-            const float gv = ffv[t][i] > 0.f ? (acc0[i] + acc1[i]) * mff.keep(kbf[t][i], D.drop_scale) : 0.f;
+        const int cu = ((32 / G) * m + T * wave + t) * 16 + li;
+        f32x4 gvv;
+#pragma unroll
+        for (int i = 0; i < 4; ++i) {
+            const float gv = kp.ffv[t][i] > 0.f ? (acc0[i] + acc1[i]) * mff.keep(kp.kbf[t][i], D.drop_scale) : 0.f;
+            gvv[i] = gv;
             if (live) D.d_ff1[(size_t)(row0 + 4 * q + i) * (4 * H) + cu] = gv;
             bf3_store1(imgF, kD3P4, 4 * q + i, cu, live ? gv : 0.f);
         }
-    }
-    __syncthreads();
-    R3D_CHAIN_MARK(D.timeline, b == 0, 12);
-    acc0 = zero; acc1 = zero;
-    bf3_chunk<4>(imgF, kD3P4, li, q, 0, b1, acc0, acc1);
-    __builtin_amdgcn_sched_barrier(0);
-    bf3_bload<4>(b1, D.pl_w1_t, 16, wave, 12, lane);
-    __builtin_amdgcn_sched_barrier(0);
-    bf3_chunk<4>(imgF, kD3P4, li, q, 4, b2, acc0, acc1);
-    __builtin_amdgcn_sched_barrier(0);
-    bf3_bload<4>(b2, D.pl_wo_t, 4, wave, 0, lane);
-    __builtin_amdgcn_sched_barrier(0);
-    bf3_chunk<4>(imgF, kD3P4, li, q, 8, b0, acc0, acc1);
-    bf3_chunk<4>(imgF, kD3P4, li, q, 12, b1, acc0, acc1);
+        if (G > 1) dx_put(x, kDxSlotDff1, cu, q, gvv);
+    }
+    if (G > 1) {
+        R3D_CHAIN_MARK(D.timeline, mk, 20);
+        dx_arrive(x, kDxDff1);
+        dx_wait(x, kDxDff1, G);
+        R3D_CHAIN_MARK(D.timeline, mk, 21);
+        dx_gather_ffn<G>(x, kDxSlotDff1, imgF, m, wave, li, q);
+    }
+    __syncthreads();
+    R3D_CHAIN_MARK(D.timeline, mk, 12);
+    f32x4 dv = zero;
+    if (own) {
+        acc0 = zero; acc1 = zero;
+#pragma unroll
+        for (int t = 0; t < 4; ++t) {
+            const int j = T + t;
+            bf3_chunk<4>(imgF, kD3P4, li, q, 4 * t, bb[j % 3], acc0, acc1);
+            __builtin_amdgcn_sched_barrier(0);
+            if (j + 3 < nc) dc3_bwd_load<G>(bb[j % 3], D, j + 3, m, wave, lane);
+            __builtin_amdgcn_sched_barrier(0);
+        }
+#pragma unroll
+        for (int i = 0; i < 4; ++i) dv[i] = live ? (acc0[i] + acc1[i]) + res[i] : 0.f;
+    }
+    if (G > 1) {
+        if (own) dx_put(x, kDxSlotD, c, q, dv);
+        R3D_CHAIN_MARK(D.timeline, mk, 22);
+        dx_arrive(x, kDxD);
+        dx_wait(x, kDxD, G);
+        R3D_CHAIN_MARK(D.timeline, mk, 23);
+        dv = dx_get(x, kDxSlotD, c, q);
+    }
     {
-        float d[4], xh[4], g[4], gx[4], s1v[4], s2v[4];
-#pragma unroll
-        for (int i = 0; i < 4; ++i) {
-            d[i] = live ? (acc0[i] + acc1[i]) + res[i] : 0.f;
-            xh[i] = (t2pv[i] - m2v[i]) * r2v[i];
+        float d[4], xh[4], g[4], s1v[4], s2v[4];
+#pragma unroll
+        for (int i = 0; i < 4; ++i) {
+#pragma clang fp contract(off)
+            d[i] = dv[i];
+            xh[i] = (kp.t2p[i] - kp.mean[i]) * kp.rstd[i];
             g[i] = d[i] * g2;
-            gx[i] = g[i] * xh[i];
-        }
+        }
+        if (live && own) {
+#pragma clang fp contract(off)
+            float* pp = D.part_d2 + (size_t)(2 * b + q) * (2 * H);
+            pp[c] = __builtin_fmaf(d[0], xh[0], d[1] * xh[1]) + __builtin_fmaf(d[2], xh[2], d[3] * xh[3]);
+            pp[H + c] = (d[0] + d[1]) + (d[2] + d[3]);
+        }
+        dc3_rowsum2(g, xh, redA, wave, li, q, s1v, s2v);
+#pragma unroll
+        for (int i = 0; i < 4; ++i) {
+#pragma clang fp contract(off)
+            const float v = kp.rstd[i] * __builtin_fmaf(-xh[i], s2v[i], g[i] - s1v[i]);
+            const size_t e = (size_t)(row0 + 4 * q + i) * H + c;
+            const float ok = v * md2.keep(kp.kb2[i], D.drop_scale);
+            if (live && own) { D.d_t2pre[e] = v; D.d_cap[e] = ok; }
+            bf3_store1(imgA, kD3P1, 4 * q + i, c, live ? ok : 0.f);
+        }
+    }
+    __syncthreads();
+    R3D_CHAIN_MARK(D.timeline, mk, 13);
+    if (own) {
+        acc0 = zero; acc1 = zero;
+        bf3_chunk<4>(imgA, kD3P1, li, q, 0, bb[(T + 4) % 3], acc0, acc1);
         if (live) {
-            float* pp = D.part_d2 + (size_t)(2 * b + q) * (2 * H);
-            pp[c] = (d[0] * xh[0] + d[1] * xh[1]) + (d[2] * xh[2] + d[3] * xh[3]);
-            pp[H + c] = (d[0] + d[1]) + (d[2] + d[3]);
-        }
-        fb_rowsum2<4>(g, gx, redA, wave, li, q, s1v, s2v);
-#pragma unroll
-        for (int i = 0; i < 4; ++i) {
-            const float o = r2v[i] * (g[i] - s1v[i] - xh[i] * s2v[i]);
-            const size_t e = (size_t)(row0 + 4 * q + i) * H + c;
-            const float ok = o * md2.keep(kb2[i], D.drop_scale);
-            if (live) { D.d_t2pre[e] = o; D.d_cap[e] = ok; }
-            bf3_store1(imgA, kD3P1, 4 * q + i, c, live ? ok : 0.f);
-        }
-    }
-    __syncthreads();
-    R3D_CHAIN_MARK(D.timeline, b == 0, 13);
-    acc0 = zero; acc1 = zero;
-    bf3_chunk<4>(imgA, kD3P1, li, q, 0, b2, acc0, acc1);
-    if (live) {
-#pragma unroll
-        for (int i = 0; i < 4; ++i) D.d_cao[(size_t)(row0 + 4 * q + i) * H + c] = acc0[i] + acc1[i];
-    }
-    R3D_CHAIN_MARK(D.timeline, b == 0, 14);
-    __syncthreads();
-    {
-        MhaArgs m{};
-        m.q = D.caq; m.ldq = H; m.k = D.cakv; m.ldk = 2 * H; m.v = D.cakv + H; m.ldv = 2 * H;
-        m.probs = D.p_ca; m.drop = D.drop_ca; m.drop_scale = D.drop_scale; m.d_o = D.d_cao; m.lddo = H;
-        m.dq = D.d_caq; m.lddq = H; m.dk = D.d_cakv; m.lddk = 2 * H; m.dv = D.d_cakv + H; m.lddv = 2 * H;
-        m.B = D.B; m.heads = 8; m.Lq = 8; m.Lk = D.S; m.dh = 16; m.scale = 0.25f;
-        mha_bwd_small_unit<16, 8, false>(m, b * 8 + wave, scr);
-    }
-    R3D_CHAIN_MARK(D.timeline, b == 0, 15);
-}
-
+#pragma unroll
+            for (int i = 0; i < 4; ++i) D.d_cao[(size_t)(row0 + 4 * q + i) * H + c] = acc0[i] + acc1[i];
+        }
+    }
+    R3D_CHAIN_MARK(D.timeline, mk, 14);
+    __syncthreads();
+    if (own) {
+        MhaArgs a{};
+        a.q = D.caq; a.ldq = H; a.k = D.cakv; a.ldk = 2 * H; a.v = D.cakv + H; a.ldv = 2 * H;
+        a.probs = D.p_ca; a.drop = D.drop_ca; a.drop_scale = D.drop_scale; a.d_o = D.d_cao; a.lddo = H;
+        a.dq = D.d_caq; a.lddq = H; a.dk = D.d_cakv; a.lddk = 2 * H; a.dv = D.d_cakv + H; a.lddv = 2 * H;
+        a.B = D.B; a.heads = 8; a.Lq = 8; a.Lk = D.S; a.dh = 16; a.scale = 0.25f;
+        mha_bwd_small_unit<16, 8, false>(a, b * 8 + wave, scr);
+    }
+    R3D_CHAIN_MARK(D.timeline, mk, 15);
+}
+
+template <int G>
 __global__ __launch_bounds__(512) void decoder_chain_bf3_kernel(const DcArgs D, const r3d_tail_losses_args t, const LossArgs a,
-                                                                float* part, unsigned* arrivals) {
+                                                                float* part, unsigned* arrivals, float* xws) {
     extern __shared__ __attribute__((aligned(16))) float lds[];
     __shared__ float lg[8][kTLHeads + 8];
     __shared__ float dl[8][kTLHeads + 8];
     __shared__ float red[8][4][128];
-    __shared__ int is_last;
+    __shared__ int is_last, fail;
     if (threadIdx.x >= 256) __builtin_amdgcn_s_setprio(0); else __builtin_amdgcn_s_setprio(2);
     const int lane = threadIdx.x & 63, wave = threadIdx.x >> 6;
-    if ((int)blockIdx.x < D.B) {
-        const int b = (int)blockIdx.x;
-        if (D.phases & 1) dc3_fwd(D, b, lds);
-        R3D_CHAIN_MARK(D.timeline, b == 0, 6);
-        if (D.phases & 2) {
-            __syncthreads();
-            tail_clip_body(t, a, part, b, lg, dl, red);
-        }
-        R3D_CHAIN_MARK(D.timeline, b == 0, 7);
-        if (D.phases & 4) {
-            __syncthreads();
-            dc3_bwd(D, b, lds);
+    const int blk = (int)blockIdx.x;
+    const int nclip = G == 1 ? D.B : (D.B + 7) / 8 * 8 * G;
+    if (blk < nclip) {
+        const int m = G == 1 ? 0 : (blk % (8 * G)) / 8;
+        const int b = G == 1 ? blk : (blk / (8 * G)) * 8 + blk % 8;
+        if (b < D.B) {
+            DcX x{};
+            if (G > 1) {
+                unsigned* xu = reinterpret_cast<unsigned*>(xws);
+                x.err = xu;
+                x.ctr = xu + kDxCtrLine * (1 + b);
+                x.slots = xws + kDxCtrLine * (1 + D.B) + (size_t)b * kDxClipFloats;
+                x.fail = &fail;
+                if (threadIdx.x == 0) fail = 0;
+            }
+            Dc3Keep<G> kp;
+            if (D.phases & 1) dc3_fwd<G>(D, b, m, lds, x, kp);
+            R3D_CHAIN_MARK(D.timeline, b == 0 && m == 0, 6);
+            if ((D.phases & 2) && m == 0) {
+                __syncthreads();
+                tail_clip_body(t, a, part, b, lg, dl, red);
+                if (G > 1 && (D.phases & 4)) {
+                    __syncthreads();
+                    dc3_publish_tail(D, b, x);
+                }
+            }
+            R3D_CHAIN_MARK(D.timeline, b == 0 && m == 0, 7);
+            if (D.phases & 4) {
+                __syncthreads();
+                dc3_bwd<G>(D, b, m, lds, x, kp, (D.phases & 1) != 0, (D.phases & 2) != 0);
+            }
+            if (G > 1 && (D.phases & 5)) dx_finish(x, G);
         }
     } else if (D.phases & 2) {
-        const int u = ((int)blockIdx.x - D.B) * 8 + wave;
+        const int u = (blk - nclip) * 8 + wave;
         if (u < a.B * a.S) losses_unit(a, part, u, lane);
     }
     if (D.phases & 2) tail_losses_finish(t, a, part, arrivals, &is_last);
@@ -591,6 +828,21 @@
 using namespace r3d;
 
 R3D_EXPORT int r3d_decoder_tail_losses_supported(int H, int n_head, int Q, int rows);
+R3D_EXPORT int64_t r3d_losses_ws_floats(int B, int S, int Q);
+
+static int dc_group_for(int B) { return B <= 32 ? 4 : (B <= 64 ? 2 : 1); }
+static int64_t dc_xoff(int B, int S, int Q) { return (r3d_losses_ws_floats(B, S, Q) + 31) / 32 * 32; }
+
+R3D_EXPORT int r3d_decoder_chain_ws_layout(int B, int S, int Q, int group, int64_t* out) {
+    R3D_REQUIRE(out && B > 0 && S > 0 && Q > 0);
+    const int G = group > 0 ? group : dc_group_for(B);
+    R3D_REQUIRE(G == 1 || G == 2 || G == 4);
+    const int64_t x = dc_xoff(B, S, Q);
+    out[0] = x + (int64_t)kDxCtrLine * (1 + B) + (G > 1 ? (int64_t)B * kDxClipFloats : 0);
+    out[1] = x;
+    out[2] = G;
+    return R3D_OK;
+}
 
 R3D_EXPORT int r3d_decoder_chain_supported(int H, int Q, int heads, int S) {
     return (H == kFcH && Q == 8 && heads == 8 && S > 0 && S <= 64) ? 1 : 0;
@@ -632,11 +884,29 @@
     }
     if (d->pl_wo) {
         R3D_REQUIRE(d->pl_w1 && d->pl_w2 && d->pl_w2_t && d->pl_w1_t && d->pl_wo_t);
-        hipError_t e3 = hipFuncSetAttribute((const void*)decoder_chain_bf3_kernel, hipFuncAttributeMaxDynamicSharedMemorySize,
-                                            kD3LdsBytes);
+        const int G = d->group > 0 ? d->group : dc_group_for(d->B);
+        R3D_REQUIRE(G == 1 || G == 2 || G == 4);
+        float* xws = nullptr;
+        if (G > 1) {
+            R3D_REQUIRE(ws);
+            if (!r3d_aligned16(ws)) return R3D_EALIGN;
+            xws = ws + dc_xoff(d->B, d->S, d->Q);
+        }
+        const int nclip = G == 1 ? d->B : r3d_cdiv(d->B, 8) * 8 * G;
+        const int grid3 = nclip + ((d->phases & 2) ? r3d_cdiv(t.B * t.S, 8) : 0);
+        const void* fn = G == 4 ? (const void*)decoder_chain_bf3_kernel<4>
+                       : G == 2 ? (const void*)decoder_chain_bf3_kernel<2> : (const void*)decoder_chain_bf3_kernel<1>;
+        hipError_t e3 = hipFuncSetAttribute(fn, hipFuncAttributeMaxDynamicSharedMemorySize, kD3LdsBytes);
         if (e3 != hipSuccess) return (int)e3;
-        hipLaunchKernelGGL(decoder_chain_bf3_kernel, dim3(grid), dim3(512), (size_t)kD3LdsBytes, (hipStream_t)stream, *d, t, a, ws,
-                           arrivals);
+        if (G == 4)
+            hipLaunchKernelGGL(decoder_chain_bf3_kernel<4>, dim3(grid3), dim3(512), (size_t)kD3LdsBytes, (hipStream_t)stream, *d, t,
+                               a, ws, arrivals, xws);
+        else if (G == 2)
+            hipLaunchKernelGGL(decoder_chain_bf3_kernel<2>, dim3(grid3), dim3(512), (size_t)kD3LdsBytes, (hipStream_t)stream, *d, t,
+                               a, ws, arrivals, xws);
+        else
+            hipLaunchKernelGGL(decoder_chain_bf3_kernel<1>, dim3(grid3), dim3(512), (size_t)kD3LdsBytes, (hipStream_t)stream, *d, t,
+                               a, ws, arrivals, xws);
         R3D_LAUNCH_CHECK();
         return R3D_OK;
     }
diff --git a/r3d_amd/engine.py b/r3d_amd/engine.py
--- a/r3d_amd/engine.py
+++ b/r3d_amd/engine.py
@@ -132,7 +132,8 @@
         self.seg = f(N, K)
         self.loss = f(4)
         self.tables = {}
-        self.loss_ws = torch.zeros(ops.losses_ws_floats(B, S, eng.Q), dtype=torch.float32, device=dev)
+        self.loss_ws = torch.zeros(max(ops.losses_ws_floats(B, S, eng.Q), ops.decoder_chain_ws_layout(B, S, eng.Q, 4)[0]),
+                                   dtype=torch.float32, device=dev)
         self.counts = torch.zeros(4, dtype=torch.int64, device=dev)
         if train:
             self.d_actdur, self.d_seg = torch.zeros(BQ, K + 1, dtype=torch.float32, device=dev), f(N, K)
@@ -193,6 +194,7 @@
         self.use_gemm_ln = True
         self.use_fuser_chain = True
         self.use_decoder_chain = True
+        self.dec_chain_group = 0
         self.chain_bf3 = True
         self._planes = None
         self.overlap_planes = False
@@ -607,7 +609,9 @@
                 w2=a.p(pl + "linear2.weight"), b2=a.p(pl + "linear2.bias"), drop_d3=dk("d3_0"), t3_pre=c["t3_pre"],
                 d_t3pre=g("t3pre"), d_ff2=g("ff2"), d_ff1=g("ff1"), d_t2pre=g("t2pre"), d_cap=g("cap"), d_cao=g("cao"),
                 d_caq=g("caq"), d_cakv=g("cakv"), part_d2=w.lnp["d2_0"] if gl is not None else None,
-                drop_scale=1.0 / (1.0 - DROP_P), pad_idx=self.pad_idx, B=w.B, S=w.S, H=H, Q=self.Q, heads=self.heads, planes=dpl)
+                drop_scale=1.0 / (1.0 - DROP_P), pad_idx=self.pad_idx, B=w.B, S=w.S, H=H, Q=self.Q, heads=self.heads, planes=dpl,
+                ws=w.loss_ws)
+        w.tables[key].args.group = int(self.dec_chain_group)
         return w.tables[key]
 
     def _gln(self, rows, K):
diff --git a/r3d_amd/ops.py b/r3d_amd/ops.py
--- a/r3d_amd/ops.py
+++ b/r3d_amd/ops.py
@@ -438,6 +438,12 @@
     return bool(_lib.load().r3d_decoder_chain_supported(H, Q, heads, S))
 
 
+def decoder_chain_ws_layout(B, S, Q, group=0):
+    out = (C.c_int64 * 3)()
+    check(_lib.load().r3d_decoder_chain_ws_layout(int(B), int(S), int(Q), int(group), out), "r3d_decoder_chain_ws_layout")
+    return int(out[0]), int(out[1]), int(out[2])
+
+
 class DecoderChain:
 
     def __init__(self, **t):
@@ -445,6 +451,11 @@
         a = DecoderChainArgs()
         dims = {k: t.pop(k) for k in ("pad_idx", "B", "S", "H", "Q", "heads")}
         a.drop_scale = float(t.pop("drop_scale", 1.0))
+        a.group = int(t.pop("group", 0))
+        self.ws = t.pop("ws", None)
+        if self.ws is not None:
+            assert self.ws.is_cuda and self.ws.dtype == torch.float32
+            assert self.ws.numel() >= decoder_chain_ws_layout(dims["B"], dims["S"], dims["Q"], a.group)[0]
         opt = {"key_label", "drop_ca", "drop_d2", "drop_ff", "drop_d3", "d_t3pre", "d_ff2", "d_ff1", "d_t2pre", "d_cap", "d_cao",
                "d_caq", "d_cakv", "part_d2"}
         planes = t.pop("planes", None)
@@ -469,6 +480,7 @@
         a = self.args
         a.phases = int(phases)
         a.key_label = None if key_label is None else key_label.data_ptr()
+        ws = self.ws if ws is None else ws
         check(_lib.load().r3d_decoder_chain(C.byref(a), C.byref(tail) if tail is not None else None, _p(ws), _stream()),
               "r3d_decoder_chain")
 
```

Result: faster. 45770 (median of 6 runs) (+3.1%).
